# ut-amrl/nautilus

Measured on AMD Instinct MI355X. Metric: loop-closure candidate pairs/sec (1081-beam), higher is better.
Workload: dtype u16

## Files before the change

nautilus_amd/csm.py:

```python
import ctypes as C
import math

import numpy as np

from . import _lib
from ._lib import GridSpec, GridLayout, Search, Match, check, ptr

MATCH_DTYPE = np.dtype([("itheta", "<i4"), ("ix", "<i4"), ("iy", "<i4"), ("score", "<f4")])
assert MATCH_DTYPE.itemsize == C.sizeof(Match) == 16


def grid_spec(range_m=30.0, res=0.05, sigma=2.0, floor_p=1e-10, max_shift=40, cell_bits=16, skip_map=False, no_image=False):
    return GridSpec(float(range_m), float(res), float(sigma), float(floor_p), int(max_shift), int(cell_bits),
                    (_lib.NHIP_GRID_SKIP_MAP if skip_map else 0) | (_lib.NHIP_GRID_NO_IMAGE if no_image else 0), 0)


def search_spec(n_theta=61, nx=81, ny=81, theta_step=math.radians(1.0), exhaustive=False, dense=False, short_scans=False,
                exact_score=False, latency=False):
    flags = (_lib.NHIP_SEARCH_EXHAUSTIVE if exhaustive else 0) | (_lib.NHIP_SEARCH_DENSE if dense else 0) | \
            (_lib.NHIP_SEARCH_SHORT_SCANS if short_scans else 0) | (_lib.NHIP_SEARCH_EXACT_SCORE if exact_score else 0) | \
            (_lib.NHIP_SEARCH_LATENCY if latency else 0)
    return Search(int(n_theta), int(nx), int(ny), flags, float(theta_step))


def grid_layout(spec):
    out = GridLayout()
    check(_lib.load().nhip_grid_layout(C.byref(spec), C.byref(out)))
    return out


def angle_mod(a):
    return a - 2.0 * math.pi * np.rint(a / (2.0 * math.pi))


def rot0_table(rot_a, rot_b=None):
    rot_a = np.ascontiguousarray(rot_a, dtype=np.float64)
    rb = None if rot_b is None else np.ascontiguousarray(rot_b, dtype=np.float64)
    out = np.empty((rot_a.size, 2), dtype=np.float64)
    check(_lib.load().nhip_csm_rot0(ptr(rot_a), ptr(rb), rot_a.size, ptr(out)))
    return out


def delta_table(search):
    out = np.empty((search.n_theta, 2), dtype=np.float64)
    check(_lib.load().nhip_csm_delta_table(C.byref(search), ptr(out)))
    return out


def pack_scans(scans):
    offsets = np.zeros(len(scans) + 1, dtype=np.int32)
    for i, s in enumerate(scans):
        offsets[i + 1] = offsets[i] + len(s)
    xy = np.zeros((int(offsets[-1]), 2), dtype=np.float32)
    for i, s in enumerate(scans):
        if len(s):
            xy[offsets[i]:offsets[i + 1]] = np.asarray(s, dtype=np.float32).reshape(-1, 2)
    return xy, offsets


class ScanTable:

    def __init__(self, xy, offsets):
        self.xy = np.ascontiguousarray(xy, dtype=np.float32).reshape(-1, 2)
        self.offsets = np.ascontiguousarray(offsets, dtype=np.int32)
        self.n_scans = self.offsets.size - 1
        self._h = C.c_void_p()
        check(_lib.load().nhip_scans_upload(ptr(self.xy), ptr(self.offsets), self.n_scans, C.byref(self._h)))

    @classmethod
    def from_list(cls, scans):
        return cls(*pack_scans(scans))

    def close(self):
        if self._h:
            _lib.load().nhip_scans_free(self._h)
            self._h = C.c_void_p()

    __del__ = close


class LikelihoodGrids:

    def __init__(self, scans, target_ids, spec):
        self.spec = spec
        self.layout = grid_layout(spec)
        self.target_ids = np.ascontiguousarray(target_ids, dtype=np.int32)
        self._h = C.c_void_p()
        check(_lib.load().nhip_grids_build(scans._h, ptr(self.target_ids), self.target_ids.size,
                                           C.byref(spec), C.byref(self._h)))

    @classmethod
    def from_submaps(cls, scans, member_scan, member_affine, member_offsets, spec):
        self = cls.__new__(cls)
        self.spec = spec
        self.layout = grid_layout(spec)
        self.member_scan = np.ascontiguousarray(member_scan, dtype=np.int32)
        self.member_affine = np.ascontiguousarray(member_affine, dtype=np.float32).reshape(-1, 4)
        self.member_offsets = np.ascontiguousarray(member_offsets, dtype=np.int32)
        if self.member_offsets.size < 1 or len(self.member_affine) != self.member_scan.size:
            raise ValueError("from_submaps: one affine per member, n_targets + 1 offsets")
        self.target_ids = np.arange(self.member_offsets.size - 1, dtype=np.int32)
        self._h = C.c_void_p()
        check(_lib.load().nhip_grids_build_submaps(scans._h, ptr(self.member_scan), ptr(self.member_affine),
                                                   ptr(self.member_offsets), self.target_ids.size, C.byref(spec),
                                                   C.byref(self._h)))
        return self

    def was_rebuilt(self):
        return bool(_lib.load().nhip_grids_was_rebuilt(self._h))

    def download(self, slot):
        L = self.layout
        out = np.empty((L.rows, L.pitch), dtype=np.uint8)
        check(_lib.load().nhip_grids_download(self._h, int(slot), ptr(out)))
        return out.view(np.uint16) if L.cell_bytes == 2 else out

    def hi_plane(self, slot, copy=0):
        L = self.layout
        out = np.empty((L.rows, L.hi_pitch), dtype=np.uint8)
        check(_lib.load().nhip_grids_download_hi_plane_copy(self._h, int(slot), int(copy), ptr(out)))
        return out

    def tiled16(self, slot):
        L = self.layout
        out = np.empty((L.rows, L.pitch), dtype=np.uint8)
        check(_lib.load().nhip_grids_download_tiled16(self._h, int(slot), ptr(out)))
        return out.view(np.uint16)

    def skip_map(self, slot):
        L = self.layout
        out = np.empty(L.skip_bytes, dtype=np.uint8)
        check(_lib.load().nhip_grids_download_skip_map(self._h, int(slot), ptr(out)))
        mp = 8 * ((L.pitch // 4 + 63) // 64)
        return out[:L.rows * mp].reshape(L.rows, mp)

    def pooled(self, slot, level=1):
        L = self.layout
        if level == 1:
            out = np.empty((L.pool_rows, L.pool_pitch), dtype=np.uint8)
            check(_lib.load().nhip_grids_download_pool(self._h, int(slot), ptr(out)))
        else:
            out = np.empty((L.pool4_rows, L.pool4_pitch), dtype=np.uint8)
            check(_lib.load().nhip_grids_download_pool4(self._h, int(slot), ptr(out)))
        return out

    def hits(self, slot):
        L = self.layout
        raw = np.empty(L.hits_bytes, dtype=np.uint8)
        check(_lib.load().nhip_grids_download_hits(self._h, int(slot), ptr(raw)))
        rows = raw[:L.hits_pitch * (L.side + 64)].reshape(L.side + 64, L.hits_pitch)
        bits = np.unpackbits(rows, axis=1, bitorder="little")
        return bits[32:32 + L.side, 32:32 + L.side]

    def interior(self, slot):
        L = self.layout
        return self.download(slot)[L.pad:L.pad + L.side, L.pad:L.pad + L.side]

    def close(self):
        if self._h:
            _lib.load().nhip_grids_free(self._h)
            self._h = C.c_void_p()

    __del__ = close


def submap_member_affines(poses, anchor_of_member, member_scan):
    P = np.ascontiguousarray(poses, dtype=np.float64).reshape(-1, 3)
    a = np.ascontiguousarray(anchor_of_member, dtype=np.int32)
    m = np.ascontiguousarray(member_scan, dtype=np.int32)
    if a.size != m.size:
        raise ValueError("submap_member_affines: one anchor per member")
    out = np.empty((m.size, 4), dtype=np.float32)
    check(_lib.load().nhip_submap_member_affines(ptr(P), len(P), ptr(a), ptr(m), m.size, ptr(out)))
    return out


def match_pairs(scans, grids, pair_src, pair_slot, theta0, search, pair_origin=None, min_score=None):
    pair_src = np.ascontiguousarray(pair_src, dtype=np.int32)
    pair_slot = np.ascontiguousarray(pair_slot, dtype=np.int32)
    theta0 = np.ascontiguousarray(theta0, dtype=np.float64)
    n = pair_src.size
    if pair_slot.size != n or theta0.size != n:
        raise ValueError("pair arrays differ in length")
    org = None
    if pair_origin is not None:
        org = np.ascontiguousarray(pair_origin, dtype=np.int32).reshape(n, 2)
    out = np.zeros(n, dtype=MATCH_DTYPE)
    sums = np.zeros(n, dtype=np.int32)
    if min_score is None:
        check(_lib.load().nhip_csm_match(scans._h, grids._h, ptr(pair_src), ptr(pair_slot), ptr(theta0),
                                         ptr(org), n, C.byref(search), ptr(out), ptr(sums)))
    else:
        check(_lib.load().nhip_csm_match_gated(scans._h, grids._h, ptr(pair_src), ptr(pair_slot), ptr(theta0),
                                               ptr(org), n, C.byref(search), ptr(out), ptr(sums), float(min_score)))
    return out, sums


def rejected(matches):
    return np.asarray(matches)["itheta"] < 0


def gate_floor(spec, min_score, n_points):
    out = C.c_int32(0)
    check(_lib.load().nhip_csm_gate_floor(C.byref(spec), float(min_score), int(n_points), C.byref(out)))
    return out.value


def bnb_stats():
    a, b = C.c_uint64(0), C.c_uint64(0)
    check(_lib.load().nhip_bnb_stats(C.byref(a), C.byref(b)))
    return a.value, b.value


def bnb_stats_levels():
    v = (C.c_uint64 * 24)()
    check(_lib.load().nhip_bnb_stats_levels(v))
    return {"blocks_whole": v[0], "blocks_total": v[1], "candidates_refined": v[2], "sub_blocks": v[3],
            "clk_wave_phase3": v[4], "clk_origins": v[5], "clk_sub_bounds": v[6], "clk_exact": v[7],
            "clk_slowest_wave": v[8], "clk_seeds": v[9], "clk_bounds": v[10], "clk_wave_phase3_100MHz": v[11],
            "pairs_handed_over": v[12], "clk_wave_second_kernel": v[13], "pose_evals16": v[14],
            "pairs_settled_by_gate": v[15], "passes_l2_runs": v[16], "passes_per_cell_field": v[17],
            "passes_per_cell_capacity": v[18]}


def score_volume(scans, grids, src, slot, theta0, search, origin=(0, 0)):
    out = np.zeros((search.n_theta, search.nx, search.ny), dtype=np.int32)
    check(_lib.load().nhip_csm_scores(scans._h, grids._h, int(src), int(slot), float(theta0),
                                      int(origin[0]), int(origin[1]), C.byref(search), ptr(out)))
    return out


def match_to_transform(m, spec, search, theta0, origin=(0, 0)):
    tx = (origin[0] + int(m["ix"]) - (search.nx - 1) // 2) * spec.res
    ty = (origin[1] + int(m["iy"]) - (search.ny - 1) // 2) * spec.res
    th = theta0 + (int(m["itheta"]) - (search.n_theta - 1) // 2) * search.theta_step
    return np.float32(tx), np.float32(ty), np.float32(th)


class CorrelativeScanMatcher:

    def __init__(self, scanner_range, trans_range, low_res, high_res, sigma=2.0, cell_bits=16):
        self.params = _lib.CsmParams(float(scanner_range), float(trans_range), float(low_res), float(high_res),
                                     float(sigma), 1e-10, int(cell_bits), 0)

    def GetTransformation(self, pointcloud_a, pointcloud_b, rotation_a, rotation_b, rotation_restriction):
        a = np.ascontiguousarray(pointcloud_a, dtype=np.float32).reshape(-1, 2)
        b = np.ascontiguousarray(pointcloud_b, dtype=np.float32).reshape(-1, 2)
        score, tx, ty, th = C.c_double(0), C.c_float(0), C.c_float(0), C.c_float(0)
        check(_lib.load().nhip_csm_get_transformation(C.byref(self.params), ptr(a), len(a), ptr(b), len(b),
                                                      float(rotation_a), float(rotation_b), float(rotation_restriction),
                                                      C.byref(score), C.byref(tx), C.byref(ty), C.byref(th)))
        return score.value, ((np.float32(tx.value), np.float32(ty.value)), np.float32(th.value))


def last_launch():
    out = (C.c_int32 * 8)()
    check(_lib.load().nhip_csm_last_launch(out))
    form = {0: "fused", 1: "split, one round", 2: "split, rounds on one stream", 3: "split, rounds overlapped on the helper stream"}
    return {"form": form.get(out[0], "?"), "form_id": out[0], "pairs_per_round": out[1], "rounds_of_state": out[2],
            "rounds": out[3], "short_scans": bool(out[4]), "hand_over_kernel": bool(out[5]), "instrumented": bool(out[6] & 1),
            "l2_runs": bool(out[6] & 2), "n_pairs": out[7]}


def drop_in_cache_stats():
    v = [C.c_int64(0) for _ in range(4)]
    check(_lib.load().nhip_csm_cache_stats(*[C.byref(x) for x in v]))
    return dict(zip(("entries", "bytes", "hits", "misses"), (x.value for x in v)))


def drop_in_cache_clear():
    check(_lib.load().nhip_csm_cache_clear())


def drop_in_cache_configure(max_bytes):
    check(_lib.load().nhip_csm_cache_configure(int(max_bytes)))
```

nautilus_amd/csrc/nhip_bnb.hip:

```cpp
#include <atomic>
#include <mutex>
#include <type_traits>
#include <vector>

#ifndef NHIP_BNB_INSTR
#define NHIP_BNB_INSTR 0
#endif
#if NHIP_BNB_INSTR
#define csm_bnb_kernel csm_bnb_kernel_instr
#define csm_bnb_rot_kernel csm_bnb_rot_kernel_instr
#define launchers_product launchers_instr
#define BNB_STATS(P) ((P).stats)
#define BNB_TIMELINE(P) ((P).timeline)
#else
#define BNB_STATS(P) (static_cast<unsigned long long *>(nullptr))
#define BNB_TIMELINE(P) (static_cast<unsigned long long *>(nullptr))
#endif

#include "nhip_bnb_params.h"
#include "nhip_bnb_wave.h"
#include "nhip_bnb_origin.h"
#include "nhip_bnb_bounds.h"
#include "nhip_bnb_exact.h"

namespace nhip {

namespace {

using namespace bnb;

constexpr int BNB_THREADS = 64 * BNB_WAVES;

struct PairCtx {
  const uint8_t *grid;
  const float2 *pts;
  int32_t n_pts, cx, cy, pair;
};

template <int CB>
__device__ __forceinline__ void process_candidate(const BnbParams &P, const PairCtx &C, int32_t k, int32_t v, int lane,
                                                  unsigned long long *best, uint32_t (&n)[4]) {
  const int Y = v / NB, X = v - NB * Y;
  float cf, sf;
  rotation_k(P, C.pair, k, &cf, &sf);
  if (P.levels >= 2) {
    const __amdgpu_buffer_rsrc_t p4 = uniform_rsrc(C.grid + P.grid_bytes + P.skip_bytes + P.pool_bytes, P.pool4_bytes);
    uint32_t sb[4];
    sub_bounds(P, p4, C.pts, C.n_pts, cf, sf, C.cx, C.cy, Y, X, lane, CB == 1 ? 1u : 257u, sb);
    n[1]++;
    const uint32_t bsum = best_sum<false>(best);
    int alive = 0;
#pragma unroll
    for (int q = 0; q < 4; q++) alive += (sb[q] != 0u && sb[q] >= bsum) ? 1 : 0;
    if (alive == 0) return;
    if (alive <= 2) {
      const __amdgpu_buffer_rsrc_t rsrc = uniform_rsrc(C.grid, P.grid_bytes + P.skip_bytes);
#pragma unroll 1
      for (int q = 0; q < 4; q++) {
        const uint32_t b = q == 0 ? sb[0] : (q == 1 ? sb[1] : (q == 2 ? sb[2] : sb[3]));
        if (b == 0u || b < best_sum<false>(best)) continue;
        const unsigned long long key = eval_sub<CB>(P, rsrc, C.pts, C.n_pts, cf, sf, C.cx, C.cy, k, Y, X, q >> 1, q & 1, lane);
        wave_atomic_max(best, key, lane);
        n[2]++;
      }
      return;
    }
  }
  const unsigned long long key = eval_block<CB>(P, C.grid, C.pts, C.n_pts, cf, sf, C.cx, C.cy, k, Y, X, lane);
  wave_atomic_max(best, key, lane);
  n[0]++;
}

template <int CB, bool GLOBAL>
__device__ __forceinline__ void process_candidate_c(const BnbParams &P, __amdgpu_buffer_rsrc_t rsrc, uint32_t pitch8,
                                                    __amdgpu_buffer_rsrc_t rsrc16, const uint32_t *org, int32_t nch,
                                                    int32_t n_pts, int32_t k, int32_t Y, int32_t X,
                                                    uint32_t sb0, uint32_t sb1, uint32_t sb2, uint32_t sb3, int lane,
                                                    unsigned long long *best, uint32_t &bcopy, uint32_t (&n)[4]) {
  const uint32_t bsum = best_sum_cached<GLOBAL>(best, bcopy);
  const int alive = (sb0 != 0u && sb0 >= bsum) + (sb1 != 0u && sb1 >= bsum) + (sb2 != 0u && sb2 >= bsum) +
                    (sb3 != 0u && sb3 >= bsum);
  if (alive == 0) return;
  constexpr int WHOLE_MIN = 3;
  if (alive >= WHOLE_MIN) {
    int dy, dx;
    const uint32_t total = block_sums8(rsrc, pitch8, (uint32_t)P.hi_copy_bytes, org, nch, Y, X, lane, &dy, &dx);
    const int32_t ix = BNB_B * X + dx, iy = BNB_B * Y + dy;
    if (CB == 1) {
      const unsigned long long key = best_key(P, k, ix, iy, total, 32);
      wave_atomic_max(best, key, lane);
      if (GLOBAL) bcopy = max(bcopy, (uint32_t)(key >> 32));
    } else {
      n[3] += refine16<GLOBAL>(P, rsrc16, org, nch, n_pts, k, ix, iy, total, true, lane, best, bcopy);
    }
    n[0]++;
    return;
  }
#pragma unroll 1
  for (int q = 0; q < 4; q++) {
    const uint32_t b = q == 0 ? sb0 : (q == 1 ? sb1 : (q == 2 ? sb2 : sb3));
    if (b == 0u || b < best_sum_cached<GLOBAL>(best, bcopy)) continue;
    int dy, dx;
    const uint32_t total = sub_sums8(rsrc, pitch8, (uint32_t)P.hi_copy_bytes, org, nch, Y, X, q >> 1, q & 1, lane, &dy, &dx);
    const int32_t ix = BNB_B * X + BNB_B4 * (q & 1) + dx, iy = BNB_B * Y + BNB_B4 * (q >> 1) + dy;
    if (CB == 1) {
      const unsigned long long key = best_key(P, k, ix, iy, total, 8);
      wave_atomic_max(best, key, lane);
      if (GLOBAL) bcopy = max(bcopy, (uint32_t)(key >> 32));
    } else {
      n[3] += refine16<GLOBAL>(P, rsrc16, org, nch, n_pts, k, ix, iy, total, lane < 16, lane, best, bcopy);
    }
    n[2]++;
  }
}

struct PhaseClocks {
  long long org, strip, eval;
  uint32_t run_passes, cell_passes_field, cell_passes_full;
};

__device__ __forceinline__ void flush_stats(unsigned long long *stats, const uint32_t *n, int32_t pair, const PhaseClocks *clk) {
  if (n) {
    if (n[0]) atomicAdd(&stats[0], (unsigned long long)n[0]);
    if (n[1]) atomicAdd(&stats[2], (unsigned long long)n[1]);
    if (n[2]) atomicAdd(&stats[3], (unsigned long long)n[2]);
    if (n[3]) atomicAdd(&stats[14], (unsigned long long)n[3]);
    if (pair < BNB_STATS_PAIRS) atomicAdd(&stats[BNB_STATS_HEAD + pair], 4ull * n[0] + n[2]);
  }
  if (clk) {
    atomicAdd(&stats[5], (unsigned long long)clk->org);
    atomicAdd(&stats[6], (unsigned long long)clk->strip);
    atomicAdd(&stats[7], (unsigned long long)clk->eval);
    if (clk->run_passes) atomicAdd(&stats[16], (unsigned long long)clk->run_passes);
    if (clk->cell_passes_field) atomicAdd(&stats[17], (unsigned long long)clk->cell_passes_field);
    if (clk->cell_passes_full) atomicAdd(&stats[18], (unsigned long long)clk->cell_passes_full);
  }
}

template <int CB, bool GLOBAL, bool RUNS = false>
__device__ __forceinline__ void rotation_pass(const BnbParams &P, const PairCtx &C, int32_t k, uint32_t u0, uint32_t u1,
                                              unsigned long long m0, unsigned long long m1, int lane,
                                              unsigned long long *best, uint32_t *done, uint32_t *org,
                                              uint32_t (&n_work)[4], PhaseClocks &clk, uint32_t *runs = nullptr) {
  long long t_mark = 0;
  float cf, sf;
  rotation_k(P, C.pair, k, &cf, &sf);
  if (BNB_STATS(P)) t_mark = clock64();
  int32_t nrc = RUNS_NONE;
  const int32_t nch = cache_origins<RUNS>(P, C.pts, C.n_pts, cf, sf, C.cx, C.cy, lane, org, true, runs, RUNS && P.l2_runs != 0, &nrc);
  if (BNB_STATS(P)) clk.org += clock64() - t_mark;
  if (RUNS && BNB_STATS(P)) {
    clk.run_passes += nrc > 0 ? 1u : 0u;
    clk.cell_passes_field += nrc == RUNS_FIELD ? 1u : 0u;
    clk.cell_passes_full += nrc == RUNS_FULL ? 1u : 0u;
  }
  const __amdgpu_buffer_rsrc_t rsrc16 = CB == 1 ? uniform_rsrc(C.grid, P.grid_bytes + P.skip_bytes)
                                                : uniform_rsrc(C.grid + P.hi_offset + 2 * P.hi_copy_bytes, P.t16_bytes);
  const __amdgpu_buffer_rsrc_t rsrc = uniform_rsrc(C.grid + P.hi_offset, 2 * P.hi_copy_bytes);
  const uint32_t pitch8 = (uint32_t)P.hi_tpr;
  const __amdgpu_buffer_rsrc_t p4 = uniform_rsrc(C.grid + P.grid_bytes + P.skip_bytes + P.pool_bytes, P.pool4_bytes);
  while ((m0 | m1) != 0ull) {
    const int b0 = m0 ? (int)__builtin_ctzll(m0) : 64 + (int)__builtin_ctzll(m1);
    const int Y = b0 / NB, X0 = b0 - NB * Y;
    int len = 1;
    while (len < 3 && X0 + len < NB) {
      const int b = b0 + len;
      if (!(((b < 64 ? m0 >> b : m1 >> (b - 64)) & 1ull))) break;
      len++;
    }
    uint32_t sb[12];
    uint32_t bcopy = GLOBAL ? best_sum<true>(best) : 0u;
    if (P.levels >= 2) {
      if (BNB_STATS(P)) t_mark = clock64();
      if (RUNS && nrc > 0) strip_bounds_c<RunList<RUN_CHUNKS>>(P, p4, runs + lane, nrc, Y, X0, len, CB == 1 ? 1u : 257u, sb);
      else strip_bounds_c<CellList>(P, p4, org, nch, Y, X0, len, CB == 1 ? 1u : 257u, sb);
      if (BNB_STATS(P)) clk.strip += clock64() - t_mark;
      n_work[1] += (uint32_t)len;
    } else {
#pragma unroll
      for (int q = 0; q < 12; q++) sb[q] = 0xffffffffu;
    }
#pragma unroll 1
    for (int t = 0; t < len; t++) {
      const int b = b0 + t;
      if (b < 64) m0 &= ~(1ull << b);
      else m1 &= ~(1ull << (b - 64));
      const uint32_t ub = (uint32_t)__builtin_amdgcn_readlane((int)(b < 64 ? u0 : u1), b & 63);
      if (ub < best_sum_cached<GLOBAL>(best, bcopy)) continue;
      const uint32_t s0 = t == 0 ? sb[0] : (t == 1 ? sb[4] : sb[8]), s1 = t == 0 ? sb[1] : (t == 1 ? sb[5] : sb[9]);
      const uint32_t s2 = t == 0 ? sb[2] : (t == 1 ? sb[6] : sb[10]), s3 = t == 0 ? sb[3] : (t == 1 ? sb[7] : sb[11]);
      if (BNB_STATS(P)) t_mark = clock64();
      process_candidate_c<CB, GLOBAL>(P, rsrc, pitch8, rsrc16, org, nch, C.n_pts, k, Y, X0 + t, s0, s1, s2, s3, lane, best,
                                      bcopy, n_work);
      if (BNB_STATS(P)) clk.eval += clock64() - t_mark;
      if (done && wave_leader(lane)) done[b] = 0u;
    }
  }
}

__device__ __forceinline__ void read_entry(const RotEntry *ent, int32_t *pair, int32_t *k, unsigned long long *m0,
                                           unsigned long long *m1) {
  const unsigned long long w0 = ent->w[0], w1 = ent->w[1], w2 = ent->w[2], w3 = ent->w[3];
  *pair = (int32_t)(w0 >> 24);
  *k = (int32_t)(w0 & 0xffffffull);
  *m0 = w1 | (w2 << 41);
  *m1 = (w2 >> 23) | (w3 << 18);
}

__device__ __forceinline__ void pair_context(const BnbParams &P, int32_t pair, PairCtx *C) {
  const int32_t src = P.pair_src[pair], slot = P.pair_slot[pair];
  const int32_t beg = P.offsets[src];
  C->grid = P.grids + (size_t)slot * P.slot_bytes;
  C->pts = P.xy + beg;
  C->n_pts = P.offsets[src + 1] - beg;
  C->cx = P.pair_origin ? P.pair_origin[2 * pair] : 0;
  C->cy = P.pair_origin ? P.pair_origin[2 * pair + 1] : 0;
  C->pair = pair;
}

template <int CB, bool POOL_LDS, bool BY_ROT, bool SPLIT = false>
__global__ __launch_bounds__(SPLIT ? 64 * SPLIT_WAVES : BNB_THREADS, SPLIT ? SPLIT_WAVES / 2 : 4) void csm_bnb_kernel(BnbParams P) {
  constexpr int WAVES = SPLIT ? SPLIT_WAVES : BNB_WAVES, THREADS = 64 * WAVES;
  constexpr int QSPACE = lds_qspace(SPLIT);
  extern __shared__ __align__(16) uint8_t smem[];
  uint8_t *s_pool = smem;
  uint32_t *s_org = reinterpret_cast<uint32_t *>(smem);
  uint32_t *s_U = reinterpret_cast<uint32_t *>(smem + P.lds_first);
  unsigned long long *s_queue = reinterpret_cast<unsigned long long *>(s_U + (size_t)P.n_theta * 128);
  LdsTail *s_tail = reinterpret_cast<LdsTail *>(s_queue + QSPACE);
  unsigned long long *s_best = &s_tail->best, *s_slow = &s_tail->slow;
  uint32_t *s_cnt = s_tail->cnt, *s_qn = s_cnt + LDS_QN, *s_qhead = s_cnt + LDS_QHEAD, *s_top = &s_tail->top;
  uint32_t *s_list = reinterpret_cast<uint32_t *>(s_queue);
  static_assert(BNB_WAVES * LIST_ENTRIES * 4 <= QCAP * 4, "the run lists fit the first half of the queue");
  unsigned long long *s_kmax = s_queue + (SPLIT ? WAVES * LIST_ENTRIES / 2 : QCAP / 2);
  uint32_t *s_order = reinterpret_cast<uint32_t *>(s_kmax + MAX_ROT);
  static_assert(SPLIT_WAVES * LIST_ENTRIES * 4 + MAX_ROT * 12 <= QSPACE_SPLIT * 8 && MAX_ROT * 12 <= QCAP * 4, "lists, maxima and order fit");

  const uint32_t bid = blockIdx.x;
  const int32_t pair = (int32_t)((bid & 7u) * (uint32_t)P.pairs_per_xcd + (bid >> 3));
  if ((int32_t)(bid >> 3) >= P.pairs_per_xcd || pair >= P.n_pairs) return;
  const int lane = threadIdx.x & 63, wave = threadIdx.x >> 6;

  int32_t src = P.pair_src[pair], slot = P.pair_slot[pair];
  const bool ids_ok = pair_ids_ok(P.ids, src, slot, pair + P.pair_base, threadIdx.x == 0);
  if (!ids_ok) src = slot = 0;
  const int32_t beg = ids_ok ? P.offsets[src] : 0, n_pts = ids_ok ? P.offsets[src + 1] - beg : 0;
  const float2 *pts = P.xy + beg;
  const uint8_t *grid = P.grids + (size_t)slot * P.slot_bytes;
  const int32_t cx = P.pair_origin ? P.pair_origin[2 * pair] : 0;
  const int32_t cy = P.pair_origin ? P.pair_origin[2 * pair + 1] : 0;
  const bool centre_ok = (abs(cx) + P.hx <= P.max_shift) && (abs(cy) + P.hy <= P.max_shift);
  if (BY_ROT != (n_pts <= 64 * OCL && (uint32_t)P.rows < ORG_LIMIT && !P.general_all)) return;

  const int32_t gfloor = gate_floor(P.gate, n_pts);
  const unsigned long long fkey = gate_floor_key(gfloor);
  unsigned long long *const stats_g = NHIP_BNB_INSTR ? P.stats : nullptr;
  const long long t_start = BNB_STATS(P) ? clock64() : 0;
  if (BNB_TIMELINE(P) && threadIdx.x == 0 && pair < BNB_STATS_PAIRS) BNB_TIMELINE(P)[4 * pair] = wall_clock64();
  if (threadIdx.x == 0) {
    *s_slow = 0ull;
    *s_best = fkey;
    s_cnt[0] = s_cnt[3] = s_cnt[4] = s_cnt[5] = 0u;
    s_top[0] = 0u;
    *s_qn = 0u;
    *s_qhead = 0u;
  }
  if (!centre_ok || n_pts <= 0) {
    if (threadIdx.x == 0) P.keys[pair] = fkey;
    return;
  }
  if (POOL_LDS) {
    const uint4 *gp = reinterpret_cast<const uint4 *>(grid + P.grid_bytes + P.skip_bytes);
    uint4 *sp = reinterpret_cast<uint4 *>(s_pool);
    const int32_t n16 = (int32_t)(P.pool_bytes / 16);
    for (int32_t i = threadIdx.x; i < n16; i += 4 * THREADS) {
      uint4 v[4];
#pragma unroll
      for (int j = 0; j < 4; j++) v[j] = gp[min(i + j * THREADS, n16 - 1)];
#pragma unroll
      for (int j = 0; j < 4; j++)
        if (i + j * THREADS < n16) sp[i + j * THREADS] = v[j];
    }
  }
  const __amdgpu_buffer_rsrc_t prs = uniform_rsrc(grid + P.grid_bytes + P.skip_bytes, P.pool_bytes);
  __syncthreads();

  const uint32_t scale = CB == 1 ? 1u : 257u;
  unsigned long long wbest = 0ull;
  for (int32_t k = wave; k < P.n_theta; k += WAVES) {
    float cf, sf;
    rotation_k(P, pair, k, &cf, &sf);
    uint32_t umax = 0u;
    uint32_t tot[2];
    coarse_rotation<POOL_LDS>(P, s_pool, prs, pts, n_pts, cf, sf, cx, cy, lane, s_list + wave * LIST_ENTRIES, tot);
    if (lane < 128 - NB * NB) s_U[k * 128 + NB * NB + lane] = 0u;
#pragma unroll
    for (int i = 0; i < 2; i++) {
      int Y, X;
      if (!slot_block(lane + 64 * i, &Y, &X)) continue;
      const uint32_t u = (Y < P.nby && X < P.nbx) ? tot[i] * scale : 0u;
      const int b = NB * Y + X;
      s_U[k * 128 + b] = u;
      umax = u > umax ? u : umax;
      const unsigned long long cand = ((unsigned long long)u << 32) | (uint32_t)((k << 8) | b);
      wbest = cand > wbest ? cand : wbest;
    }
    if (BY_ROT) {
      umax = wave_max(umax);
      if (wave_leader(lane)) s_kmax[k] = ((unsigned long long)umax << 32) | (uint32_t)k;
    }
  }
  wbest = wave_max_u64(wbest);
  if (gfloor > 0) {
    if (wave_leader(lane)) atomicMax(s_top, (uint32_t)(wbest >> 32));
    __syncthreads();
    if (*s_top < (uint32_t)gfloor) {
      if (threadIdx.x == 0) {
        P.keys[pair] = fkey;
        if (stats_g) {
          atomicAdd(&stats_g[1], (unsigned long long)(P.n_theta * P.nbx * P.nby));
          atomicAdd(&stats_g[15], 1ull);
        }
      }
      return;
    }
    if ((uint32_t)(wbest >> 32) < (uint32_t)gfloor) wbest = 0ull;
  }
  uint32_t n_work[4] = {0u, 0u, 0u, 0u};
  PairCtx C;
  C.grid = grid;
  C.pts = pts;
  C.n_pts = n_pts;
  C.cx = cx;
  C.cy = cy;
  C.pair = pair;
  if (BY_ROT) {
    __syncthreads();
    uint32_t *org = s_org + wave * ORG_WAVE + lane;
    PhaseClocks clk = {0, 0, 0, 0u, 0u, 0u};
    long long t_busy = 0, t_wall = 0;
    const long long t_phase1 = BNB_STATS(P) ? clock64() : 0;
    if (BNB_TIMELINE(P) && threadIdx.x == 0 && pair < BNB_STATS_PAIRS) BNB_TIMELINE(P)[4 * pair + 1] = wall_clock64();
    const uint32_t xcd = bid & 7u;
    bool handed_over = false;
    enum { SEED, OWN };
    int state = SEED;
    bool heavy = false;
    for (;;) {
      bool have = false;
      int32_t k = 0;
      uint32_t u0 = 0u, u1 = 0u;
      unsigned long long m0 = 0ull, m1 = 0ull;
      uint32_t *done = nullptr;
      if (state == SEED) {
        if ((uint32_t)(wbest >> 32) != 0u) {
          const int32_t v = (int32_t)(wbest & 0xffu);
          const uint32_t ub = (uint32_t)(wbest >> 32);
          k = (int32_t)((uint32_t)wbest >> 8);
          u0 = v == lane ? ub : 0u;
          u1 = v == lane + 64 ? ub : 0u;
          m0 = v < 64 ? 1ull << v : 0ull;
          m1 = v < 64 ? 0ull : 1ull << (v - 64);
          done = s_U + k * 128;
          have = true;
        }
      } else if (state == OWN) {
        const int32_t rank = (int32_t)wave_fetch_add(s_qhead, 1u, lane);
        if (rank >= P.n_theta) break;
        k = (int32_t)s_order[rank];
        u0 = s_U[k * 128 + lane];
        u1 = s_U[k * 128 + 64 + lane];
        const uint32_t bsum = best_sum<false>(s_best);
        m0 = __ballot(u0 != 0u && u0 >= bsum);
        m1 = __ballot(u1 != 0u && u1 >= bsum && lane + 64 < NB * NB);
        if ((m0 | m1) == 0ull) continue;
        if (heavy && (uint32_t)rank >= P.keep_ranks) {
          const uint32_t lx = (xcd + (uint32_t)rank) & 7u;
          const uint32_t e = wave_fetch_add(P.rot_count + 8 * lx, 1u, lane);
          if (e < P.rot_cap) {
            if (lane < 4) {
              const unsigned long long M41 = (1ull << 41) - 1ull;
              const unsigned long long word = lane == 0   ? ((unsigned long long)(uint32_t)pair << 24) | (uint32_t)k
                                              : lane == 1 ? (m0 & M41)
                                              : lane == 2 ? ((m0 >> 41) | (m1 << 23)) & M41
                                                          : (m1 >> 18);
              P.rot_list[(size_t)lx * P.rot_cap + e].w[lane] = word;
            }
            handed_over = true;
            continue;
          }
        }
        have = true;
      }
      if (have) rotation_pass<CB, false>(P, C, k, u0, u1, m0, m1, lane, s_best, done, org, n_work, clk);
      if (state == SEED) {
        __syncthreads();
        if (BNB_TIMELINE(P) && threadIdx.x == 0 && pair < BNB_STATS_PAIRS) BNB_TIMELINE(P)[4 * pair + 2] = wall_clock64();
        if (BNB_STATS(P)) {
          t_busy = clock64();
          t_wall = wall_clock64();
        }
        for (int32_t kk = threadIdx.x; kk < P.n_theta; kk += THREADS) {
          const unsigned long long mine = s_kmax[kk];
          int32_t rank = 0;
          for (int32_t j = 0; j < P.n_theta; j++) rank += s_kmax[j] > mine ? 1 : 0;
          s_order[rank] = (uint32_t)kk;
        }
        if (P.rot_list || SPLIT) {
          const uint32_t bsum = best_sum<false>(s_best);
          uint32_t mine = 0u;
          for (int32_t kk = wave; kk < P.n_theta; kk += WAVES) {
            const uint32_t c0 = s_U[kk * 128 + lane], c1 = s_U[kk * 128 + 64 + lane];
            mine += (uint32_t)__builtin_popcountll(__ballot(c0 != 0u && c0 >= bsum)) +
                    (uint32_t)__builtin_popcountll(__ballot(c1 != 0u && c1 >= bsum && lane + 64 < NB * NB));
          }
          if (wave_leader(lane)) atomicAdd(s_qn, mine);
        }
        __syncthreads();
        if (SPLIT) {
          const uint32_t bsum = best_sum<false>(s_best);
          uint32_t *rows = P.ps_rows + (size_t)pair * (size_t)P.n_theta * 128u;
          uint32_t live = 0u;
          for (int32_t r = wave; r < P.n_theta; r += WAVES) {
            const uint32_t kk = s_order[r];
            const uint32_t kmax = (uint32_t)(s_kmax[kk] >> 32);
            if (kmax == 0u || kmax < bsum) break;
            live = (uint32_t)r + 1u;
            const uint32_t w1 = lane == 62 ? kmax : (lane == 63 ? kk : s_U[kk * 128 + 64 + lane]);
            rows[(size_t)r * 128u + lane] = s_U[kk * 128 + lane];
            rows[(size_t)r * 128u + 64 + lane] = w1;
          }
          if (live && wave_leader(lane)) atomicMax(s_qhead, live);
          __syncthreads();
          if (threadIdx.x == 0) {
            P.ps_count[pair] = *s_qn;
            P.ps_live[pair] = *s_qhead;
            P.ps_next[pair] = 0u;
          }
          break;
        }
        heavy = P.rot_list && *s_qn >= P.heavy_min;
        state = OWN;
      }
    }
    if (BNB_STATS(P) && lane == 0) {
      const long long now = clock64();
      atomicAdd(&BNB_STATS(P)[4], (unsigned long long)(now - t_busy));
      atomicAdd(&BNB_STATS(P)[11], (unsigned long long)(wall_clock64() - t_wall));
      flush_stats(BNB_STATS(P), nullptr, pair, &clk);
      atomicMax(s_slow, (unsigned long long)(now - t_busy));
      if (wave == 0) {
        atomicAdd(&BNB_STATS(P)[9], (unsigned long long)(t_busy - t_phase1));
        atomicAdd(&BNB_STATS(P)[10], (unsigned long long)(t_phase1 - t_start));
        if (handed_over) atomicAdd(&BNB_STATS(P)[12], 1ull);
      }
    }
  } else {
  if ((uint32_t)(wbest >> 32) != 0u) {
      const int32_t k = (int32_t)((uint32_t)wbest >> 8), v = (int32_t)(wbest & 0xffu);
      const int Y = v / NB, X = v - NB * Y;
      float cf, sf;
      rotation_k(P, pair, k, &cf, &sf);
      const unsigned long long key = eval_block<CB>(P, grid, pts, n_pts, cf, sf, cx, cy, k, Y, X, lane);
      if (wave_leader(lane)) {
        atomicMax(s_best, key);
        s_U[k * 128 + v] = 0u;
      }
      n_work[0]++;
    }
    __syncthreads();
    for (int32_t k = wave; k < P.n_theta; k += BNB_WAVES) {
  #pragma unroll
      for (int i = 0; i < 2; i++) {
        const uint32_t u = s_U[k * 128 + lane + 64 * i];
        const uint32_t bsum = (uint32_t)(*(volatile unsigned long long *)s_best >> 32);
        bool cand = u != 0u && u >= bsum;
        const unsigned long long m = __ballot(cand);
        if (m == 0ull) continue;
        const uint32_t base = wave_fetch_add(s_qn, (uint32_t)__builtin_popcountll(m), lane);
        const uint32_t pos = base + (uint32_t)__builtin_popcountll(m & ((1ull << lane) - 1ull));
        const unsigned long long entry = ((unsigned long long)u << 32) | (uint32_t)((k << 8) | (lane + 64 * i));
        if (cand && pos < (uint32_t)QCAP) s_queue[pos] = entry;
        unsigned long long over = __ballot(cand && pos >= (uint32_t)QCAP);
        while (over) {
          const int j = (int)__builtin_ctzll(over);
          over &= over - 1ull;
          const uint32_t lo = (uint32_t)__builtin_amdgcn_readlane((int)(uint32_t)entry, j);
          const uint32_t hi = (uint32_t)__builtin_amdgcn_readlane((int)(uint32_t)(entry >> 32), j);
          if (hi >= best_sum<false>(s_best))
            process_candidate<CB>(P, C, (int32_t)(lo >> 8), (int32_t)(lo & 0xffu), lane, s_best, n_work);
        }
      }
    }
    __syncthreads();
    {
      const uint32_t qn = min(*s_qn, (uint32_t)QCAP);
      for (;;) {
        const uint32_t i = wave_fetch_add(s_qhead, 1u, lane);
        if (i >= qn) break;
        const unsigned long long entry = s_queue[i];
        if ((uint32_t)(entry >> 32) >= best_sum<false>(s_best))
          process_candidate<CB>(P, C, (int32_t)((uint32_t)entry >> 8), (int32_t)(entry & 0xffu), lane, s_best, n_work);
      }
    }
}
  if (stats_g && lane == 0) {
    atomicAdd(&s_cnt[0], n_work[0]);
    atomicAdd(&s_cnt[3], n_work[1]);
    atomicAdd(&s_cnt[4], n_work[2]);
    atomicAdd(&s_cnt[5], n_work[3]);
  }
  __syncthreads();
  if (threadIdx.x == 0) {
    P.keys[pair] = *s_best;
    if (BNB_TIMELINE(P) && pair < BNB_STATS_PAIRS) {
      uint32_t hw;
      asm volatile("s_getreg_b32 %0, hwreg(HW_REG_HW_ID)" : "=s"(hw));
      uint32_t xcc;
      asm volatile("s_getreg_b32 %0, hwreg(HW_REG_XCC_ID)" : "=s"(xcc));
      BNB_TIMELINE(P)[4 * pair + 3] = (wall_clock64() & 0xfffffffffffull) | ((unsigned long long)((hw >> 8) & 0xffu) << 44) |
                                      ((unsigned long long)(xcc & 0xfu) << 52);
    }
    if (BNB_STATS(P) && BY_ROT) atomicAdd(&BNB_STATS(P)[8], *s_slow);
    if (stats_g) {
      const uint32_t n_all[4] = {s_cnt[0], s_cnt[3], s_cnt[4], s_cnt[5]};
      flush_stats(stats_g, n_all, pair, nullptr);
      atomicAdd(&stats_g[1], (unsigned long long)(P.n_theta * P.nbx * P.nby));
    }
  }
}

template <int CB>
__global__ __launch_bounds__(256, 4) void csm_bnb_rot_kernel(BnbParams P) {
  const int lane = threadIdx.x & 63;
  const uint32_t xcd = blockIdx.x & 7u;
  const uint32_t filled = P.rot_count[8 * xcd];
  const uint32_t count = filled < P.rot_cap ? filled : P.rot_cap;
  const RotEntry *list = P.rot_list + (size_t)xcd * P.rot_cap;
  __shared__ uint32_t s_org2[4 * ORG_WAVE];
  __shared__ uint32_t s_run2[4 * RUN_WAVE];
  uint32_t *org = s_org2 + (threadIdx.x >> 6) * ORG_WAVE + lane;
  uint32_t *runs = s_run2 + (threadIdx.x >> 6) * RUN_WAVE;
  PhaseClocks clk = {0, 0, 0, 0u, 0u, 0u};
  const long long t0 = BNB_STATS(P) ? clock64() : 0;
  for (;;) {
    const uint32_t i = wave_fetch_add(P.rot_count + 8 * xcd + 1, 1u, lane);
    if (i >= count) break;
    int32_t pair, k;
    unsigned long long m0, m1;
    read_entry(list + i, &pair, &k, &m0, &m1);
    PairCtx C;
    pair_context(P, pair, &C);
    uint32_t n[4] = {0u, 0u, 0u, 0u};
    rotation_pass<CB, true, true>(P, C, k, 0xffffffffu, 0xffffffffu, m0, m1, lane, &P.keys[pair], nullptr, org, n, clk, runs);
    if (BNB_STATS(P) && lane == 0) flush_stats(BNB_STATS(P), n, pair, nullptr);
  }
  if (BNB_STATS(P) && lane == 0) {
    atomicAdd(&BNB_STATS(P)[13], (unsigned long long)(clock64() - t0));
    flush_stats(BNB_STATS(P), nullptr, 0, &clk);
  }
}

constexpr int SORT_THREADS = 1024;
constexpr int SORT_BUCKETS = 16 * 21;
__device__ __forceinline__ int cand_bucket(uint32_t c) {
  if (c == 0u) return SORT_BUCKETS - 1;
  const int e = 31 - __builtin_clz(c);
  const int f = e >= 4 ? (int)((c >> (e - 4)) & 15u) : (int)((c << (4 - e)) & 15u);
  const int b = 16 * e + f;
  return b >= SORT_BUCKETS - 1 ? 0 : SORT_BUCKETS - 2 - b;
}
__device__ __forceinline__ uint32_t cand_shares(const BnbParams &P, uint32_t c) {
  const uint32_t w = 1u + c / P.split_min;
  return w < P.split_max ? w : P.split_max;
}

__global__ __launch_bounds__(SORT_THREADS) void csm_bnb_order_kernel(BnbParams P) {
  __shared__ uint32_t s_extra[SORT_BUCKETS];
  __shared__ uint32_t s_wave[SORT_THREADS / 64];
  __shared__ uint32_t s_base, s_idle;
  __shared__ int s_grant;
  const int32_t xcd = blockIdx.x;
  const int32_t lo = xcd * P.pairs_per_xcd, hi = min(lo + P.pairs_per_xcd, P.n_pairs);
  int32_t *work = P.ps_work + (size_t)xcd * P.ps_work_stride;
  for (int i = threadIdx.x; i < SORT_BUCKETS; i += SORT_THREADS) s_extra[i] = 0u;
  for (int i = threadIdx.x; i < P.ps_work_stride; i += SORT_THREADS) work[i] = -1;
  if (threadIdx.x == 0) s_base = s_idle = 0u;
  __syncthreads();
  for (int32_t p = lo + (int32_t)threadIdx.x; p < hi; p += SORT_THREADS) {
    const uint32_t c = P.ps_count[p];
    atomicAdd(&s_extra[cand_bucket(c)], cand_shares(P, c) - 1u);
  }
  __syncthreads();
  if (threadIdx.x == 0) {
    uint32_t room = (uint32_t)P.ps_work_stride - (uint32_t)(hi > lo ? hi - lo : 0);
    int grant = 0;
    while (grant < SORT_BUCKETS && s_extra[grant] <= room) room -= s_extra[grant++];
    s_grant = grant;
  }
  __syncthreads();
  const int lane = threadIdx.x & 63, wv = threadIdx.x >> 6;
  for (int pass = P.front_min ? 0 : 1; pass < 2; pass++)
  for (int32_t p0 = lo; p0 < hi; p0 += SORT_THREADS) {
    const int32_t p = p0 + (int32_t)threadIdx.x;
    const uint32_t c = p < hi ? P.ps_count[p] : 0u;
    const bool mine = P.front_min == 0u || ((c >= P.front_min) == (pass == 0));
    const uint32_t w = (c != 0u && mine) ? (cand_bucket(c) < s_grant ? cand_shares(P, c) : 1u) : 0u;
    if (p < hi && mine) P.ps_nw[p] = c != 0u ? w : 1u;
    uint32_t v = w;
#pragma unroll
    for (int off = 1; off < 64; off <<= 1) {
      const uint32_t u = (uint32_t)__shfl_up((int)v, off, 64);
      if (lane >= off) v += u;
    }
    if (lane == 63) s_wave[wv] = v;
    __syncthreads();
    uint32_t before = s_base;
    for (int q = 0; q < wv; q++) before += s_wave[q];
    const uint32_t at = before + v - w;
    for (uint32_t j = 0; j < w; j++) work[at + j] = p;
    __syncthreads();
    if (threadIdx.x == SORT_THREADS - 1) s_base = before + v;
    __syncthreads();
  }
  const uint32_t tail0 = s_base;
  for (int32_t p = lo + (int32_t)threadIdx.x; p < hi; p += SORT_THREADS)
    if (P.ps_count[p] == 0u) work[tail0 + atomicAdd(&s_idle, 1u)] = p;
}

constexpr int ORDER_THREADS = 256;
__global__ __launch_bounds__(ORDER_THREADS) void csm_bnb_order_spread_kernel(BnbParams P) {
  const int32_t p = (int32_t)(blockIdx.x * ORDER_THREADS + threadIdx.x);
  if (p >= P.n_pairs) return;
  const int32_t extra_slots = P.ps_work_stride - P.pairs_per_xcd;
  const int32_t home = p / P.pairs_per_xcd;
  P.ps_work[(size_t)home * P.ps_work_stride + extra_slots + (p - home * P.pairs_per_xcd)] = p;
  const uint32_t want = cand_shares(P, P.ps_count[p]) - 1u;
  uint32_t got = 0u;
  if (want) {
    const uint32_t t0 = atomicAdd(P.ps_ticket, want);
    for (uint32_t j = 0; j < want; j++) {
      const uint32_t e = t0 + j;
      if ((int32_t)(e >> 3) >= extra_slots) break;
      P.ps_work[(size_t)((e + (uint32_t)home + 1u) & 7u) * P.ps_work_stride + (e >> 3)] = p;
      got++;
    }
  }
  P.ps_nw[p] = 1u + got;
}

constexpr int CAND_WAVES = 4;
constexpr int CAND_THREADS = 64 * CAND_WAVES;
template <int CB>
__global__ __launch_bounds__(CAND_THREADS, CB == 2 ? 5 : 4) void csm_bnb_cand_kernel(BnbParams P) {
  __shared__ uint32_t s_org2[CAND_WAVES * ORG_WAVE];
  __shared__ uint32_t s_run2[CAND_WAVES * RUN_WAVE];
  __shared__ unsigned long long s_best2;
  __shared__ uint32_t s_next2;
  const int lane = threadIdx.x & 63;
  const uint32_t xcd = blockIdx.x & 7u, slot = blockIdx.x >> 3;
  if ((int32_t)slot >= P.ps_work_stride) return;
  const int32_t pair = P.ps_work[(size_t)xcd * P.ps_work_stride + slot];
  if (pair < 0) return;
  const uint32_t live = P.ps_live[pair];
  if (live == 0u) return;
  const bool shared = P.ps_nw[pair] > 1u;
  if (BNB_TIMELINE(P) && threadIdx.x == 0 && pair < BNB_STATS_PAIRS)
    atomicMin(&BNB_TIMELINE(P)[4 * (size_t)BNB_STATS_PAIRS + 2 + pair], wall_clock64());
  if (threadIdx.x == 0) {
    s_best2 = P.keys[pair];
    s_next2 = 0u;
  }
  __syncthreads();
  unsigned long long *best = shared ? &P.keys[pair] : &s_best2;
  uint32_t *next = shared ? &P.ps_next[pair] : &s_next2;
  const uint32_t *rows = P.ps_rows + (size_t)pair * (size_t)P.n_theta * 128u;
  uint32_t *org = s_org2 + (threadIdx.x >> 6) * ORG_WAVE + lane;
  uint32_t *runs = s_run2 + (threadIdx.x >> 6) * RUN_WAVE;
  PairCtx C;
  pair_context(P, pair, &C);
  uint32_t n_work[4] = {0u, 0u, 0u, 0u};
  PhaseClocks clk = {0, 0, 0, 0u, 0u, 0u};
  const long long t0 = BNB_STATS(P) ? clock64() : 0;
  for (;;) {
    const uint32_t rank = wave_fetch_add(next, 1u, lane);
    if (rank >= live) break;
    const uint32_t u0 = rows[(size_t)rank * 128u + lane], u1 = rows[(size_t)rank * 128u + 64 + lane];
    const uint32_t kmax = (uint32_t)__builtin_amdgcn_readlane((int)u1, 62);
    const int32_t k = __builtin_amdgcn_readlane((int)u1, 63);
    const uint32_t bsum = best_sum<true>(best);
    if (kmax < bsum) break;
    const unsigned long long m0 = __ballot(u0 != 0u && u0 >= bsum);
    const unsigned long long m1 = __ballot(u1 != 0u && u1 >= bsum && lane + 64 < NB * NB);
    if ((m0 | m1) == 0ull) continue;
    rotation_pass<CB, true, true>(P, C, k, u0, u1, m0, m1, lane, best, nullptr, org, n_work, clk, runs);
  }
  if (BNB_STATS(P) && lane == 0) {
    atomicAdd(&BNB_STATS(P)[13], (unsigned long long)(clock64() - t0));
    flush_stats(BNB_STATS(P), n_work, pair, &clk);
  }
  if (BNB_TIMELINE(P) && lane == 0 && pair < BNB_STATS_PAIRS)
    atomicMax(&BNB_TIMELINE(P)[5 * (size_t)BNB_STATS_PAIRS + 2 + pair], wall_clock64());
  if (!shared) {
    __syncthreads();
    if (threadIdx.x == 0) P.keys[pair] = s_best2;
  }
}

}

namespace bnb {

namespace {
template <int CB, bool PL, bool BR, bool SP = false>
int launch_main(const BnbParams &P, const BnbPlan &plan, hipStream_t s) {
  constexpr int THREADS = SP ? 64 * SPLIT_WAVES : BNB_THREADS;
  const size_t lds = lds_bytes((size_t)plan.lds_first, P.n_theta, SP);
  const int64_t blocks = (int64_t)P.pairs_per_xcd * 8;
  constexpr int MAX_DEV = 64;
  static std::atomic<size_t> lds_set[MAX_DEV];
  int dev = 0;
  if (hipGetDevice(&dev) != hipSuccess || dev < 0 || dev >= MAX_DEV) dev = -1;
  if (dev < 0 || lds > lds_set[dev].load(std::memory_order_relaxed)) {
    NHIP_TRY_HIP(hipFuncSetAttribute(reinterpret_cast<const void *>(csm_bnb_kernel<CB, PL, BR, SP>),
                                     hipFuncAttributeMaxDynamicSharedMemorySize, (int)lds));
    if (dev >= 0) lds_set[dev].store(lds, std::memory_order_relaxed);
  }
  hipLaunchKernelGGL((csm_bnb_kernel<CB, PL, BR, SP>), dim3((uint32_t)blocks), dim3(THREADS), lds, s, P);
  return NHIP_OK;
}

template <int CB, bool PL>
int launch_split_a(const BnbParams &P, const BnbPlan &plan, hipStream_t s) {
  int rc = launch_main<CB, PL, true, true>(P, plan, s);
  if (rc) return rc;
  if (!P.short_scans && (rc = launch_main<CB, PL, false>(P, plan, s))) return rc;
  if (P.ps_ticket)
    hipLaunchKernelGGL(csm_bnb_order_spread_kernel, dim3((uint32_t)((P.n_pairs + ORDER_THREADS - 1) / ORDER_THREADS)), dim3(ORDER_THREADS), 0, s, P);
  else
    hipLaunchKernelGGL(csm_bnb_order_kernel, dim3(8), dim3(SORT_THREADS), 0, s, P);
  return NHIP_OK;
}

template <int CB, bool PL>
int launch_both(const BnbParams &P, const BnbPlan &plan, hipStream_t s) {
  if (!P.general_all) {
    int rc = launch_main<CB, PL, true>(P, plan, s);
    if (rc) return rc;
    if (P.short_scans) return NHIP_OK;
  }
  return launch_main<CB, PL, false>(P, plan, s);
}

template <class F>
int with_instantiation(const BnbPlan &plan, F f) {
  using CB1 = std::integral_constant<int, 1>;
  using CB2 = std::integral_constant<int, 2>;
  if (plan.cb == 1) return plan.pool_lds ? f(CB1{}, std::true_type{}) : f(CB1{}, std::false_type{});
  return plan.pool_lds ? f(CB2{}, std::true_type{}) : f(CB2{}, std::false_type{});
}

int launch_fused(const BnbParams &P, const BnbPlan &plan, hipStream_t s) {
  return with_instantiation(plan, [&](auto cb, auto pl) {
    const int rc = launch_both<decltype(cb)::value, decltype(pl)::value>(P, plan, s);
    if (rc) return rc;
    if (plan.second) {
      const uint32_t rot_blocks = 256 * 4;
      hipLaunchKernelGGL(csm_bnb_rot_kernel<decltype(cb)::value>, dim3(rot_blocks), dim3(256), 0, s, P);
    }
    return NHIP_OK;
  });
}

int launch_split_bounds(const BnbParams &P, const BnbPlan &plan, hipStream_t s) {
  return with_instantiation(plan, [&](auto cb, auto pl) { return launch_split_a<decltype(cb)::value, decltype(pl)::value>(P, plan, s); });
}

int launch_split_cands(const BnbParams &P, const BnbPlan &plan, hipStream_t s) {
  return with_instantiation(plan, [&](auto cb, auto) {
    hipLaunchKernelGGL(csm_bnb_cand_kernel<decltype(cb)::value>, dim3((uint32_t)(8 * P.ps_work_stride)), dim3(CAND_THREADS), 0, s, P);
    return NHIP_OK;
  });
}
}

BnbLaunchers launchers_product() { return {launch_fused, launch_split_bounds, launch_split_cands}; }

}


}
```

nautilus_amd/csrc/nhip_bnb_bounds.h:

```cpp
#pragma once
#include <type_traits>

#include "nhip_bnb_origin.h"

namespace nhip {
namespace {

constexpr uint32_t LANE_WEIGHT = 64u;

template <bool POOL_LDS>
__device__ __forceinline__ void coarse_rotation(const BnbParams &P, const uint8_t *pool, __amdgpu_buffer_rsrc_t prs,
                                                const float2 *pts, int32_t n_pts, float cf, float sf, int32_t cx,
                                                int32_t cy, int lane, uint32_t *list, uint32_t (&tot)[2]) {
  const int32_t DP = P.pool_pitch;
  const uint32_t zero_a = (uint32_t)(((P.rows + BNB_B - 1) / BNB_B) * DP);
  tot[0] = tot[1] = 0u;
  uint32_t E[NB][3], O[NB][3];
#pragma unroll
  for (int y = 0; y < NB; y++)
#pragma unroll
    for (int d = 0; d < 3; d++) E[y][d] = O[y][d] = 0u;
  uint32_t head = 0u, tail = 0u;
  uint32_t reduced = 0u;
  uint32_t weight = 0u;

  auto gather = [&](uint32_t a, uint32_t cnt) {
    const uint32_t se = __umul24(a & 3u, 0x10001u) + 0x0c020c00u, so = se + 0x00010001u;
    const uint32_t *q = reinterpret_cast<const uint32_t *>(pool + (a & ~3u));
#pragma unroll
    for (int y = 0; y < NB; y++) {
      uint32_t w0, w1, w2, w3;
      if (POOL_LDS) {
        const uint32_t *row = q + (y * DP) / 4;
        w0 = row[0]; w1 = row[1]; w2 = row[2]; w3 = row[3];
      } else {
        const u32x4 r4 = __builtin_amdgcn_raw_buffer_load_b128(prs, (int)((a & ~3u) + (uint32_t)(y * DP)), 0, 0);
        w0 = r4.x; w1 = r4.y; w2 = r4.z; w3 = r4.w;
      }
      E[y][0] += __umul24(__builtin_amdgcn_perm(w1, w0, se), cnt); O[y][0] += __umul24(__builtin_amdgcn_perm(w1, w0, so), cnt);
      E[y][1] += __umul24(__builtin_amdgcn_perm(w2, w1, se), cnt); O[y][1] += __umul24(__builtin_amdgcn_perm(w2, w1, so), cnt);
      E[y][2] += __umul24(__builtin_amdgcn_perm(w3, w2, se), cnt); O[y][2] = mad24(__builtin_amdgcn_perm(w3, w2, so), cnt, O[y][2]);
    }
  };
  auto reduce = [&]() {
    uint32_t R[64];
#pragma unroll
    for (int y = 0; y < 10; y++)
#pragma unroll
      for (int d = 0; d < 3; d++) {
        R[6 * y + d] = E[y][d];
        R[6 * y + 3 + d] = O[y][d];
      }
    R[5] = (O[0][2] & 0xffffu) | (O[10][1] << 16);
    R[11] = (O[1][2] & 0xffffu) | (O[10][1] & 0xffff0000u);
    R[17] = (O[2][2] & 0xffffu) | (O[10][2] << 16);
    R[60] = E[10][0];
    R[61] = E[10][1];
    R[62] = E[10][2];
    R[63] = O[10][0];
    rs_step<64, 1>(R, lane & 1);
    rs_step<32, 2>(R, lane & 2);
    uint32_t V[32];
#pragma unroll
    for (int i = 0; i < 16; i++) {
      V[2 * i] = R[i] & 0xffffu;
      V[2 * i + 1] = R[i] >> 16;
    }
    rs_step<32, 4>(V, lane & 4);
    rs_step<16, 8>(V, lane & 8);
    rs_step<8, 16>(V, lane & 16);
    rs_step<4, 32>(V, lane & 32);
    tot[0] += V[0];
    tot[1] += V[1];
#pragma unroll
    for (int y = 0; y < NB; y++)
#pragma unroll
      for (int d = 0; d < 3; d++) E[y][d] = O[y][d] = 0u;
  };

  auto feed = [&](uint32_t a, int32_t c, bool more) {
    if (more) {
      const bool live = c + lane < n_pts;
      const uint32_t prev = (uint32_t)__builtin_amdgcn_update_dpp((int)a, (int)a, 0x138 , 0xF, 0xF, false);
      const bool is_head = (lane & 63) == 0 || a != prev;
      const unsigned long long H = __builtin_amdgcn_uicmp(a, prev, 33 ) | 1ull;
      uint32_t cnt = (uint32_t)(c + lane) & 127u;
      cnt += 1u;
      const int32_t n_live = n_pts - c;
      const unsigned long long He = H & (n_live >= 64 ? ~0ull : (1ull << n_live) - 1ull);
      if (is_head && live) {
        const uint32_t before = __builtin_amdgcn_mbcnt_hi((uint32_t)(He >> 32), __builtin_amdgcn_mbcnt_lo((uint32_t)He, 0u));
        list[(tail + before) & (LIST_ENTRIES - 1)] = a | ((cnt - 1u) << RUN_SHIFT);
      }
      tail += (uint32_t)__builtin_popcountll(He);
      __builtin_amdgcn_fence(__ATOMIC_RELEASE, "wavefront");
      __builtin_amdgcn_wave_barrier();
    }
    if (!more) {
      if (lane == 0) list[tail & (LIST_ENTRIES - 1)] = ((uint32_t)n_pts & 127u) << RUN_SHIFT;
      __builtin_amdgcn_fence(__ATOMIC_RELEASE, "wavefront");
      __builtin_amdgcn_wave_barrier();
    }
    for (;;) {
      const uint32_t avail = tail - head;
      if (avail < 65u && more) break;
      const bool last = avail == 0u;
      const bool mine = (uint32_t)lane < avail;
      const uint32_t entry = mine ? list[(head + (uint32_t)lane) & (LIST_ENTRIES - 1)] : zero_a;
      const uint32_t ea = entry & ((1u << RUN_SHIFT) - 1u);
      const uint32_t next = mine ? list[(head + (uint32_t)lane + 1u) & (LIST_ENTRIES - 1)] : 0u;
      const uint32_t cnt = mine ? ((next >> RUN_SHIFT) - (entry >> RUN_SHIFT)) & 127u : 0u;
      uint32_t left = avail;
      asm("" : "+s"(left));
      if (head != reduced && (left == 0u || __builtin_amdgcn_uicmp(weight + cnt, LANE_WEIGHT, 34 ) != 0ull)) {
        reduce();
        reduced = head;
        weight = 0u;
      }
      if (last) break;
      gather(ea, cnt);
      weight += cnt;
      head += avail < 64u ? avail : 64u;
      __builtin_amdgcn_wave_barrier();
    }
  };

  auto offsets = [&](float2 pt, int32_t c) {
    uint32_t a = zero_a;
    if (c + lane < n_pts) {
      int32_t prow, pcol;
      window_origin<true>(pt, cf, sf, P, cx, cy, &prow, &pcol);
      a = __umul24((uint32_t)prow >> 3, (uint32_t)DP) + ((uint32_t)pcol >> 3);
    }
    return a;
  };
  constexpr int PD = 2;
  if (n_pts > 0) {
    const int32_t last = n_pts - 1;
    float2 q0 = pts[min(lane, last)];
    __builtin_amdgcn_sched_barrier(0);
    float2 q1 = pts[min(64 + lane, last)];
    for (int32_t c = 0; c < n_pts; c += 64 * PD) {
      {
        float2 pt = q0;
        asm volatile("" : "+v"(pt.x), "+v"(pt.y));
        q0 = pts[min(c + 64 * PD + lane, last)];
        feed(offsets(pt, c), c, true);
      }
      {
        float2 pt = q1;
        asm volatile("" : "+v"(pt.x), "+v"(pt.y));
        q1 = pts[min(c + 64 * PD + 64 + lane, last)];
        if (c + 64 < n_pts) feed(offsets(pt, c + 64), c + 64, true);
      }
    }
  }
  feed(zero_a, 0, false);
}

__device__ __forceinline__ bool slot_block(int v, int *Y, int *X) {
  const int lane = v & 63, i = v >> 6;
  const int r = 32 * i + 16 * ((lane >> 5) & 1) + 8 * ((lane >> 4) & 1) + 4 * ((lane >> 3) & 1) + 2 * ((lane >> 1) & 1) + (lane & 1);
  const int f = (lane >> 2) & 1;
  if (r >= 60) {
    *Y = 10;
    *X = r == 63 ? 1 + 2 * f : 4 * (r - 60) + 2 * f;
    return true;
  }
  const int y = r / 6, d = r % 6;
  if (d == 5 && f == 1) {
    *Y = 10;
    *X = 5 + 2 * y;
    return y < 3;
  }
  *Y = y;
  *X = d < 3 ? 4 * d + 2 * f : 4 * (d - 3) + 1 + 2 * f;
  return true;
}

__device__ __forceinline__ void sub_bounds(const BnbParams &P, __amdgpu_buffer_rsrc_t p4, const float2 *pts, int32_t n_pts,
                                           float cf, float sf, int32_t cx, int32_t cy, int32_t Y, int32_t X, int lane,
                                           uint32_t scale, uint32_t (&out)[4]) {
  const int32_t DP = P.pool4_pitch;
  uint32_t A[4] = {0u, 0u, 0u, 0u};
  constexpr int U = 4;
  for (int32_t c = 0; c < n_pts; c += 64 * U) {
    uint32_t a[U];
    u32x2 w[U];
#pragma unroll
    for (int u = 0; u < U; u++) {
      const int32_t idx = c + 64 * u + lane;
      a[u] = 0u;
      if (idx < n_pts) {
        int32_t prow, pcol;
        window_origin(pts[idx], cf, sf, P, cx, cy, &prow, &pcol);
        a[u] = (uint32_t)(((prow >> 2) + 2 * Y) * DP + 2 * ((pcol >> 2) + 2 * X));
      }
      w[u] = __builtin_amdgcn_raw_buffer_load_b64(p4, (int)(a[u] & ~3u), 0, 0);
    }
#pragma unroll
    for (int u = 0; u < U; u++) {
      const uint32_t n = idx_guard(c + 64 * u + lane < n_pts, __builtin_amdgcn_alignbit(w[u].y, w[u].x, (a[u] & 2u) * 8u));
      A[0] += n & 0xffu;
      A[2] += (n >> 8) & 0xffu;
      A[1] += (n >> 16) & 0xffu;
      A[3] += n >> 24;
    }
  }
#pragma unroll
  for (int m = 1; m < 64; m <<= 1) {
#pragma unroll
    for (int q = 0; q < 4; q++) A[q] += shfl_xor_u32(A[q], m);
  }
#pragma unroll
  for (int q = 0; q < 4; q++) out[q] = A[q] * scale;
}

struct CellList {
  static constexpr int ROUNDS = 2, H = OC / ROUNDS;
  static __device__ __forceinline__ uint32_t entry(const uint32_t *list, int c) { return origin_of(list, c); }
  static __device__ __forceinline__ uint32_t offset(uint32_t o, uint32_t DP) { return (org_row(o) >> 2) * DP + 2u * (org_col(o) >> 2); }
  static __device__ __forceinline__ uint32_t count(uint32_t o) { return org_cnt(o); }
};
template <int CHUNKS>
struct RunList {
  static constexpr int ROUNDS = 1, H = CHUNKS;
  static __device__ __forceinline__ uint32_t entry(const uint32_t *list, int c) { return list[64 * c]; }
  static __device__ __forceinline__ uint32_t offset(uint32_t e, uint32_t DP) { return run_row2(e) * DP + 2u * run_col2(e); }
  static __device__ __forceinline__ uint32_t count(uint32_t e) { return run_cnt(e); }
};

template <class LIST>
__device__ __forceinline__ void strip_sums(const BnbParams &P, __amdgpu_buffer_rsrc_t p4, const uint32_t *list, int32_t nch,
                                           int32_t Y, int32_t X0, int len, uint32_t (&E)[3], uint32_t (&O)[3]) {
  const uint32_t DP = (uint32_t)P.pool4_pitch;
  const uint32_t off = (uint32_t)(2 * Y) * DP + (uint32_t)(4 * X0);
  constexpr int ROUNDS = LIST::ROUNDS, H = LIST::H;
#pragma unroll
  for (int h = 0; h < ROUNDS; h++) {
    if (H * h >= nch) continue;
    u32x4 w[H];
    uint32_t sh[H], cn[H];
    uint32_t aa[H];
#pragma unroll
    for (int j = 0; j < H; j++) {
      const uint32_t o = LIST::entry(list, H * h + j);
      const uint32_t a = LIST::offset(o, DP) + off;
      sh[j] = (a & 2u) * 8u;
      aa[j] = a & ~3u;
      cn[j] = LIST::count(o);
    }
    if (len == 1) {
#pragma unroll
      for (int j = 0; j < H; j++) {
        const u32x2 v = __builtin_amdgcn_raw_buffer_load_b64(p4, (int)aa[j], 0, 0);
        w[j].x = v.x; w[j].y = v.y; w[j].z = 0u; w[j].w = 0u;
      }
    } else if (len == 2) {
#pragma unroll
      for (int j = 0; j < H; j++) {
        const u32x3 v = __builtin_amdgcn_raw_buffer_load_b96(p4, (int)aa[j], 0, 0);
        w[j].x = v.x; w[j].y = v.y; w[j].z = v.z; w[j].w = 0u;
      }
    } else {
#pragma unroll
      for (int j = 0; j < H; j++) w[j] = __builtin_amdgcn_raw_buffer_load_b128(p4, (int)aa[j], 0, 0);
    }
#pragma unroll
    for (int j = 0; j < H; j++) {
      const uint32_t n0 = __builtin_amdgcn_alignbit(w[j].y, w[j].x, sh[j]);
      const uint32_t n1 = __builtin_amdgcn_alignbit(w[j].z, w[j].y, sh[j]);
      const uint32_t n2 = __builtin_amdgcn_alignbit(w[j].w, w[j].z, sh[j]);
      E[0] += __umul24(n0 & M8, cn[j]); O[0] += __umul24((n0 >> 8) & M8, cn[j]);
      E[1] += __umul24(n1 & M8, cn[j]); O[1] += __umul24((n1 >> 8) & M8, cn[j]);
      E[2] += __umul24(n2 & M8, cn[j]); O[2] += __umul24((n2 >> 8) & M8, cn[j]);
    }
  }
}

template <class LIST>
__device__ __forceinline__ void strip_bounds_c(const BnbParams &P, __amdgpu_buffer_rsrc_t p4, const uint32_t *list,
                                               int32_t nch, int32_t Y, int32_t X0, int len, uint32_t scale,
                                               uint32_t (&out)[12]) {
  uint32_t E[3] = {0u, 0u, 0u}, O[3] = {0u, 0u, 0u};
  if (std::is_same<LIST, CellList>::value) {
    strip_sums<CellList>(P, p4, list, nch, Y, X0, len, E, O);
  } else {
    static_assert(RUN_CHUNKS == 8, "the rounds below cover the run list");
    if (nch <= 4) strip_sums<RunList<4>>(P, p4, list, nch, Y, X0, len, E, O);
    else if (nch == 5) strip_sums<RunList<5>>(P, p4, list, nch, Y, X0, len, E, O);
    else if (nch == 6) strip_sums<RunList<6>>(P, p4, list, nch, Y, X0, len, E, O);
    else strip_sums<RunList<8>>(P, p4, list, nch, Y, X0, len, E, O);
  }
#pragma unroll
  for (int t = 0; t < 3; t++) {
    E[t] = sum8(E[t]);
    O[t] = sum8(O[t]);
  }
#pragma unroll
  for (int t = 0; t < 3; t++) {
    out[4 * t + 0] = E[t] & 0xffffu;
    out[4 * t + 1] = E[t] >> 16;
    out[4 * t + 2] = O[t] & 0xffffu;
    out[4 * t + 3] = O[t] >> 16;
  }
#pragma unroll
  for (int q = 0; q < 12; q++) out[q] = wave_total_of8(out[q]) * scale;
}

}
}
```

nautilus_amd/csrc/nhip_bnb_exact.h:

```cpp
#pragma once
#include "nhip_bnb_origin.h"

namespace nhip {
namespace {

constexpr int SEG_CHUNKS = 32;
constexpr int EVAL_CHUNKS = 2;

template <bool GLOBAL>
__device__ __forceinline__ uint32_t best_sum(unsigned long long *best) {
  unsigned long long b;
  if (GLOBAL) b = __hip_atomic_load(best, __ATOMIC_RELAXED, __HIP_MEMORY_SCOPE_AGENT);
  else b = *(volatile unsigned long long *)best;
  return (uint32_t)__builtin_amdgcn_readfirstlane((int)(uint32_t)(b >> 32));
}
template <bool GLOBAL>
__device__ __forceinline__ uint32_t best_sum_cached(unsigned long long *best, uint32_t copy) {
  return GLOBAL ? copy : best_sum<false>(best);
}

__device__ __forceinline__ unsigned long long best_key(const BnbParams &P, int32_t k, int32_t ix, int32_t iy, uint32_t total,
                                                       int top) {
  unsigned long long key = 0ull;
  if (ix < P.nx && iy < P.ny) {
    const uint32_t lin = (uint32_t)((k * P.nx + ix) * P.ny + iy);
    key = ((unsigned long long)total << 32) | (0xffffffffu - lin);
  }
#pragma unroll
  for (int m = 32; m >= 1; m >>= 1) {
    if (m > top) continue;
    const unsigned long long o = shfl_xor_u64b(key, m);
    key = o > key ? o : key;
  }
  return key;
}

template <int CB>
__device__ __forceinline__ unsigned long long eval_block(const BnbParams &P, const uint8_t *grid, const float2 *pts,
                                                         int32_t n_pts, float cf, float sf, int32_t cx, int32_t cy,
                                                         int32_t k, int32_t Y, int32_t X, int lane) {
  uint32_t total = 0u;
  int dy, dx;
  const __amdgpu_buffer_rsrc_t rsrc = uniform_rsrc(grid, P.grid_bytes + P.skip_bytes);
  if (CB == 1) {
    const float2 none = make_float2(0.f, 0.f);
    for (int32_t c0 = 0; c0 < n_pts; c0 += 64 * SEG_CHUNKS) {
      uint32_t E[8][2], O[8][2];
#pragma unroll
      for (int y = 0; y < 8; y++) E[y][0] = E[y][1] = O[y][0] = O[y][1] = 0u;
      const int32_t c1 = min(n_pts, c0 + 64 * SEG_CHUNKS);
      float qx[EVAL_CHUNKS], qy[EVAL_CHUNKS];
#pragma unroll
      for (int u = 0; u < EVAL_CHUNKS; u++) {
        const float2 q = c0 + 64 * u + lane < c1 ? pts[c0 + 64 * u + lane] : none;
        qx[u] = q.x;
        qy[u] = q.y;
      }
      for (int32_t c = c0; c < c1; c += 64 * EVAL_CHUNKS) {
        float nx[EVAL_CHUNKS], ny[EVAL_CHUNKS];
#pragma unroll
        for (int u = 0; u < EVAL_CHUNKS; u++) {
          const int32_t idx = c + 64 * (EVAL_CHUNKS + u) + lane;
          const float2 q = idx < c1 ? pts[idx] : none;
          nx[u] = q.x;
          ny[u] = q.y;
        }
        uint32_t g[EVAL_CHUNKS], sh[EVAL_CHUNKS], w[EVAL_CHUNKS][8][3];
#pragma unroll
        for (int u = 0; u < EVAL_CHUNKS; u++) {
          const int32_t idx = c + 64 * u + lane;
          patch_origin(P, idx < c1, make_float2(qx[u], qy[u]), cf, sf, cx, cy, Y, X, &g[u], &sh[u]);
#pragma unroll
          for (int y = 0; y < 8; y++) {
            const u32x3 r = __builtin_amdgcn_raw_buffer_load_b96(rsrc, (int)(g[u] + (uint32_t)(y * P.pitch)), 0, 0);
            w[u][y][0] = r.x; w[u][y][1] = r.y; w[u][y][2] = r.z;
          }
        }
#pragma unroll
        for (int u = 0; u < EVAL_CHUNKS; u++) {
#pragma unroll
          for (int y = 0; y < 8; y++) {
            const uint32_t n0 = __builtin_amdgcn_alignbit(w[u][y][1], w[u][y][0], sh[u]);
            const uint32_t n1 = __builtin_amdgcn_alignbit(w[u][y][2], w[u][y][1], sh[u]);
            E[y][0] += n0 & M8; O[y][0] += n0 >> 8;
            E[y][1] += n1 & M8; O[y][1] += n1 >> 8;
          }
          qx[u] = nx[u];
          qy[u] = ny[u];
        }
      }
      uint32_t R[32];
#pragma unroll
      for (int y = 0; y < 8; y++) {
        R[4 * y + 0] = E[y][0];
        R[4 * y + 1] = O[y][0] - ((E[y][0] >> 16) << 8);
        R[4 * y + 2] = E[y][1];
        R[4 * y + 3] = O[y][1] - ((E[y][1] >> 16) << 8);
      }
      rs_step<32, 1>(R, lane & 1);
      rs_step<16, 2>(R, lane & 2);
      rs_step<8, 4>(R, lane & 4);
      uint32_t V[8];
#pragma unroll
      for (int i = 0; i < 4; i++) {
        V[2 * i] = R[i] & 0xffffu;
        V[2 * i + 1] = R[i] >> 16;
      }
      rs_step<8, 8>(V, lane & 8);
      rs_step<4, 16>(V, lane & 16);
      rs_step<2, 32>(V, lane & 32);
      total += V[0];
    }
    const int r = 8 * (2 * ((lane >> 5) & 1) + ((lane >> 4) & 1)) + 4 * ((lane >> 2) & 1) + 2 * ((lane >> 1) & 1) + (lane & 1);
    const int f = (lane >> 3) & 1, d = r & 3;
    dy = r >> 2;
    dx = 4 * (d >> 1) + (d & 1) + 2 * f;
  } else {
    uint32_t A[64];
#pragma unroll
    for (int i = 0; i < 64; i++) A[i] = 0u;
    float2 qn = lane < n_pts ? pts[lane] : make_float2(0.f, 0.f);
    for (int32_t c = 0; c < n_pts; c += 64) {
      const float2 q = qn;
      if (c + 64 + lane < n_pts) qn = pts[c + 64 + lane];
      uint32_t g = 0u, sh = 0u;
      if (c + lane < n_pts) {
        int32_t prow, pcol;
        window_origin(q, cf, sf, P, cx, cy, &prow, &pcol);
        const int32_t col = pcol + BNB_B * X;
        g = (uint32_t)((prow + BNB_B * Y) * P.pitch + ((2 * col) & ~3));
        sh = (uint32_t)(col & 1) * 16u;
      }
#pragma unroll
      for (int y = 0; y < 8; y++) {
        const u32x4 r4 = __builtin_amdgcn_raw_buffer_load_b128(rsrc, (int)(g + (uint32_t)(y * P.pitch)), 0, 0);
        const uint32_t w[5] = {r4.x, r4.y, r4.z, r4.w,
                               __builtin_amdgcn_raw_buffer_load_b32(rsrc, (int)(g + (uint32_t)(y * P.pitch) + 16u), 0, 0)};
#pragma unroll
        for (int j = 0; j < 4; j++) {
          const uint32_t nj = __builtin_amdgcn_alignbit(w[j + 1], w[j], sh);
          A[8 * y + 2 * j] += nj & 0xffffu;
          A[8 * y + 2 * j + 1] += nj >> 16;
        }
      }
    }
    rs_step<64, 1>(A, lane & 1);
    rs_step<32, 2>(A, lane & 2);
    rs_step<16, 4>(A, lane & 4);
    rs_step<8, 8>(A, lane & 8);
    rs_step<4, 16>(A, lane & 16);
    rs_step<2, 32>(A, lane & 32);
    total = A[0];
    dy = lane >> 3;
    dx = lane & 7;
  }
  const int32_t ix = BNB_B * X + dx, iy = BNB_B * Y + dy;
  unsigned long long key = 0ull;
  if (ix < P.nx && iy < P.ny) {
    const uint32_t lin = (uint32_t)((k * P.nx + ix) * P.ny + iy);
    key = ((unsigned long long)total << 32) | (0xffffffffu - lin);
  }
#pragma unroll
  for (int m = 32; m >= 1; m >>= 1) {
    const unsigned long long o = shfl_xor_u64b(key, m);
    key = o > key ? o : key;
  }
  return key;
}

template <int CB>
__device__ __forceinline__ unsigned long long eval_sub(const BnbParams &P, __amdgpu_buffer_rsrc_t rsrc, const float2 *pts,
                                                       int32_t n_pts, float cf, float sf, int32_t cx, int32_t cy,
                                                       int32_t k, int32_t Y, int32_t X, int32_t sy, int32_t sx, int lane) {
  uint32_t total = 0u;
  int dy, dx;
  const float2 none = make_float2(0.f, 0.f);
  constexpr int U = 4;
  if (CB == 1) {
    static_assert(SEG_CHUNKS % U == 0, "segments are whole iterations");
    for (int32_t c0 = 0; c0 < n_pts; c0 += 64 * SEG_CHUNKS) {
      uint32_t E[4], O[4];
#pragma unroll
      for (int y = 0; y < 4; y++) E[y] = O[y] = 0u;
      const int32_t c1 = min(n_pts, c0 + 64 * SEG_CHUNKS);
      for (int32_t c = c0; c < c1; c += 64 * U) {
        uint32_t sh[U];
        u32x2 w[U][4];
#pragma unroll
        for (int u = 0; u < U; u++) {
          const int32_t idx = c + 64 * u + lane;
          uint32_t g;
          patch_origin(P, idx < c1, idx < c1 ? pts[idx] : none, cf, sf, cx, cy, Y, X, &g, &sh[u]);
          if (idx < c1) g += (uint32_t)(BNB_B4 * sy * P.pitch + BNB_B4 * sx);
#pragma unroll
          for (int y = 0; y < 4; y++) w[u][y] = __builtin_amdgcn_raw_buffer_load_b64(rsrc, (int)(g + (uint32_t)(y * P.pitch)), 0, 0);
        }
#pragma unroll
        for (int u = 0; u < U; u++)
#pragma unroll
          for (int y = 0; y < 4; y++) {
            const uint32_t n = __builtin_amdgcn_alignbit(w[u][y].y, w[u][y].x, sh[u]);
            E[y] += n & M8;
            O[y] += n >> 8;
          }
      }
      uint32_t R[8];
#pragma unroll
      for (int y = 0; y < 4; y++) {
        R[2 * y] = E[y];
        R[2 * y + 1] = O[y] - ((E[y] >> 16) << 8);
      }
      rs_step<8, 1>(R, lane & 1);
      rs_step<4, 2>(R, lane & 2);
      rs_step<2, 4>(R, lane & 4);
      uint32_t V[2] = {R[0] & 0xffffu, R[0] >> 16};
      rs_step<2, 8>(V, lane & 8);
      V[0] = add_xor<16>(V[0]);
      V[0] = add_xor<32>(V[0]);
      total += V[0];
    }
    dy = ((lane >> 1) & 1) + 2 * ((lane >> 2) & 1);
    dx = (lane & 1) + 2 * ((lane >> 3) & 1);
  } else {
    uint32_t A[16];
#pragma unroll
    for (int i = 0; i < 16; i++) A[i] = 0u;
    for (int32_t c = 0; c < n_pts; c += 64 * U) {
      uint32_t sh[U];
      u32x3 w[U][4];
#pragma unroll
      for (int u = 0; u < U; u++) {
        const int32_t idx = c + 64 * u + lane;
        uint32_t g = 0u;
        sh[u] = 0u;
        if (idx < n_pts) {
          int32_t prow, pcol;
          window_origin(pts[idx], cf, sf, P, cx, cy, &prow, &pcol);
          const int32_t col = pcol + BNB_B * X + BNB_B4 * sx;
          g = (uint32_t)((prow + BNB_B * Y + BNB_B4 * sy) * P.pitch + ((2 * col) & ~3));
          sh[u] = (uint32_t)(col & 1) * 16u;
        }
#pragma unroll
        for (int y = 0; y < 4; y++) w[u][y] = __builtin_amdgcn_raw_buffer_load_b96(rsrc, (int)(g + (uint32_t)(y * P.pitch)), 0, 0);
      }
#pragma unroll
      for (int u = 0; u < U; u++)
#pragma unroll
        for (int y = 0; y < 4; y++) {
          const uint32_t n0 = __builtin_amdgcn_alignbit(w[u][y].y, w[u][y].x, sh[u]);
          const uint32_t n1 = __builtin_amdgcn_alignbit(w[u][y].z, w[u][y].y, sh[u]);
          A[4 * y + 0] += n0 & 0xffffu;
          A[4 * y + 1] += n0 >> 16;
          A[4 * y + 2] += n1 & 0xffffu;
          A[4 * y + 3] += n1 >> 16;
        }
    }
    rs_step<16, 1>(A, lane & 1);
    rs_step<8, 2>(A, lane & 2);
    rs_step<4, 4>(A, lane & 4);
    rs_step<2, 8>(A, lane & 8);
    A[0] = add_xor<16>(A[0]);
    A[0] = add_xor<32>(A[0]);
    total = A[0];
    dy = (lane >> 2) & 3;
    dx = lane & 3;
  }
  const int32_t ix = BNB_B * X + BNB_B4 * sx + dx, iy = BNB_B * Y + BNB_B4 * sy + dy;
  unsigned long long key = 0ull;
  if (ix < P.nx && iy < P.ny) {
    const uint32_t lin = (uint32_t)((k * P.nx + ix) * P.ny + iy);
    key = ((unsigned long long)total << 32) | (0xffffffffu - lin);
  }
#pragma unroll
  for (int m = 8; m >= 1; m >>= 1) {
    const unsigned long long o = shfl_xor_u64b(key, m);
    key = o > key ? o : key;
  }
  return key;
}

__device__ __forceinline__ uint32_t sub_sums8(__amdgpu_buffer_rsrc_t rsrc, uint32_t pitch, uint32_t copy_bytes, const uint32_t *org,
                                              int32_t nch, int32_t Y, int32_t X, int32_t sy, int32_t sx, int lane, int *dy, int *dx) {
  const uint32_t roff = (uint32_t)(BNB_B * Y + BNB_B4 * sy), coff = (uint32_t)(BNB_B * X + BNB_B4 * sx);
  const uint32_t wrap = pitch * HI_TILE_BYTES - HI_TILE_BYTES;
  constexpr int U = 2;
  static_assert(OC % U == 0, "whole rounds");
  uint32_t E[4] = {0u, 0u, 0u, 0u}, O[4] = {0u, 0u, 0u, 0u};
#pragma unroll
  for (int r = 0; r < OC / U; r++) {
    if (U * r >= nch) continue;
    u32x2 w[U][4];
    uint32_t sh[U], cn[U];
#pragma unroll
    for (int j = 0; j < U; j++) {
      const uint32_t o = origin_of(org, U * r + j);
      cn[j] = org_cnt(o);
      const uint32_t row0 = org_row(o) + roff, col0 = org_col(o) + coff, col4 = col0 & ~3u;
      const uint32_t cp = (col4 >> 3) & 1u, q = row0 & 7u;
      const uint32_t v0 = hi_tiled(row0, col4, cp, pitch, copy_bytes);
      sh[j] = (col0 & 3u) * 8u;
#pragma unroll
      for (int y = 0; y < 4; y++)
        w[j][y] = __builtin_amdgcn_raw_buffer_load_b64(rsrc, (int)(v0 + (q + (uint32_t)y >= 8u ? wrap : 0u) + 16u * (uint32_t)y), 0, 0);
    }
#pragma unroll
    for (int j = 0; j < U; j++)
#pragma unroll
      for (int y = 0; y < 4; y++) {
        const uint32_t n = __builtin_amdgcn_alignbit(w[j][y].y, w[j][y].x, sh[j]);
        E[y] += __umul24(n & M8, cn[j]);
        O[y] += __umul24(n >> 8, cn[j]);
      }
  }
  uint32_t R[8];
#pragma unroll
  for (int y = 0; y < 4; y++) {
    R[2 * y] = E[y];
    R[2 * y + 1] = O[y] - ((E[y] >> 16) << 8);
  }
  rs_step<8, 1>(R, lane & 1);
  rs_step<4, 2>(R, lane & 2);
  rs_step<2, 4>(R, lane & 4);
  uint32_t V[2] = {R[0] & 0xffffu, R[0] >> 16};
  rs_step<2, 8>(V, lane & 8);
  V[0] = add_xor<16>(V[0]);
  V[0] = add_xor<32>(V[0]);
  *dy = ((lane >> 1) & 1) + 2 * ((lane >> 2) & 1);
  *dx = (lane & 1) + 2 * ((lane >> 3) & 1);
  return V[0];
}

__device__ __forceinline__ uint32_t block_sums8(__amdgpu_buffer_rsrc_t rsrc, uint32_t pitch, uint32_t copy_bytes, const uint32_t *org,
                                                int32_t nch, int32_t Y, int32_t X, int lane, int *dy, int *dx) {
  const uint32_t roff = (uint32_t)(BNB_B * Y), coff = (uint32_t)(BNB_B * X);
  const uint32_t wrap = pitch * HI_TILE_BYTES - HI_TILE_BYTES;
  constexpr int U = 1;
  uint32_t E[8][2], O[8][2];
#pragma unroll
  for (int y = 0; y < 8; y++) E[y][0] = E[y][1] = O[y][0] = O[y][1] = 0u;
#pragma unroll
  for (int r = 0; r < OC / U; r++) {
    if (U * r >= nch) continue;
    constexpr int ROWS = 4;
    uint32_t gg[U], sh[U], cn[U], qq[U];
#pragma unroll
    for (int j = 0; j < U; j++) {
      const uint32_t o = origin_of(org, U * r + j);
      cn[j] = org_cnt(o);
      const uint32_t row0 = org_row(o) + roff, col0 = org_col(o) + coff, col4 = col0 & ~3u;
      qq[j] = row0 & 7u;
      gg[j] = hi_tiled(row0, col4, (col4 >> 3) & 1u, pitch, copy_bytes);
      sh[j] = (col0 & 3u) * 8u;
    }
#pragma unroll
    for (int y0 = 0; y0 < 8; y0 += ROWS) {
      u32x3 w[U][ROWS];
#pragma unroll
      for (int j = 0; j < U; j++)
#pragma unroll
        for (int y = 0; y < ROWS; y++)
          w[j][y] = __builtin_amdgcn_raw_buffer_load_b96(rsrc, (int)(gg[j] + (qq[j] + (uint32_t)(y0 + y) >= 8u ? wrap : 0u) + 16u * (uint32_t)(y0 + y)), 0, 0);
#pragma unroll
      for (int j = 0; j < U; j++)
#pragma unroll
        for (int y = 0; y < ROWS; y++) {
          const uint32_t n0 = __builtin_amdgcn_alignbit(w[j][y].y, w[j][y].x, sh[j]);
          const uint32_t n1 = __builtin_amdgcn_alignbit(w[j][y].z, w[j][y].y, sh[j]);
          E[y0 + y][0] += __umul24(n0 & M8, cn[j]); O[y0 + y][0] += __umul24(n0 >> 8, cn[j]);
          E[y0 + y][1] += __umul24(n1 & M8, cn[j]); O[y0 + y][1] += __umul24(n1 >> 8, cn[j]);
        }
    }
  }
  uint32_t R[32];
#pragma unroll
  for (int y = 0; y < 8; y++) {
    R[4 * y + 0] = E[y][0];
    R[4 * y + 1] = O[y][0] - ((E[y][0] >> 16) << 8);
    R[4 * y + 2] = E[y][1];
    R[4 * y + 3] = O[y][1] - ((E[y][1] >> 16) << 8);
  }
  rs_step<32, 1>(R, lane & 1);
  rs_step<16, 2>(R, lane & 2);
  rs_step<8, 4>(R, lane & 4);
  uint32_t V[8];
#pragma unroll
  for (int i = 0; i < 4; i++) {
    V[2 * i] = R[i] & 0xffffu;
    V[2 * i + 1] = R[i] >> 16;
  }
  rs_step<8, 8>(V, lane & 8);
  rs_step<4, 16>(V, lane & 16);
  rs_step<2, 32>(V, lane & 32);
  const int r = 8 * (2 * ((lane >> 5) & 1) + ((lane >> 4) & 1)) + 4 * ((lane >> 2) & 1) + 2 * ((lane >> 1) & 1) + (lane & 1);
  const int f = (lane >> 3) & 1, d = r & 3;
  *dy = r >> 2;
  *dx = 4 * (d >> 1) + (d & 1) + 2 * f;
  return V[0];
}

__device__ __forceinline__ uint32_t pose_sum16(const BnbParams &P, __amdgpu_buffer_rsrc_t rsrc16, const uint32_t *org,
                                               int32_t nch, int32_t ix, int32_t iy) {
  uint32_t acc = 0u;
#pragma unroll
  for (int c = 0; c < OCL; c++) {
    if (c >= nch) continue;
    const uint32_t o = origin_of(org, c);
    acc += org_cnt(o) * (uint32_t)__builtin_amdgcn_raw_buffer_load_b16(
                            rsrc16, (int)t16_tiled(org_row(o) + (uint32_t)iy, org_col(o) + (uint32_t)ix, (uint32_t)P.t16_tpr), 0, 0);
  }
  return wave_sum(acc);
}

template <bool GLOBAL>
__device__ __forceinline__ uint32_t refine16(const BnbParams &P, __amdgpu_buffer_rsrc_t rsrc16, const uint32_t *org,
                                             int32_t nch, int32_t n_pts, int32_t k, int32_t ix, int32_t iy, uint32_t hsum,
                                             bool mine, int lane, unsigned long long *best, uint32_t &bcopy) {
  const bool valid = mine && ix < P.nx && iy < P.ny;
  uint32_t ub = valid ? 256u * hsum + 255u * (uint32_t)n_pts : 0u;
  uint32_t n_eval = 0u;
  for (;;) {
    const uint32_t top = (uint32_t)__builtin_amdgcn_readfirstlane((int)wave_max(ub));
    if (top == 0u || top < best_sum_cached<GLOBAL>(best, bcopy)) break;
    const int j = (int)__builtin_ctzll(__ballot(ub == top));
    const int32_t jx = __builtin_amdgcn_readlane(ix, j), jy = __builtin_amdgcn_readlane(iy, j);
    const uint32_t sum = pose_sum16(P, rsrc16, org, nch, jx, jy);
    const uint32_t lin = (uint32_t)((k * P.nx + jx) * P.ny + jy);
    const unsigned long long key = ((unsigned long long)sum << 32) | (0xffffffffu - lin);
    wave_atomic_max(best, key, lane);
    if (GLOBAL) bcopy = max(bcopy, sum);
    if (lane == j) ub = 0u;
    n_eval++;
  }
  return n_eval;
}

}
}
```

nautilus_amd/csrc/nhip_bnb_host.hip:

```cpp
#include <atomic>
#include <memory>
#include <mutex>
#include <vector>

#include "nhip_bnb_params.h"

namespace nhip {

using namespace bnb;

namespace {

size_t bnb_lds_first(const GridLayout &L, bool pool_lds) {
  const size_t pool = pool_lds ? (size_t)L.pool_bytes : 0;
  return pool > (size_t)ORG_LDS ? pool : (size_t)ORG_LDS;
}
size_t bnb_lds_bytes(const GridLayout &L, const nhip_search_t *search, bool pool_lds) {
  return lds_bytes(bnb_lds_first(L, pool_lds), search->n_theta, false);
}
constexpr size_t LDS_MAX = 160 * 1024;

struct TimerScope {
  int id;
  hipStream_t s;
  TimerScope(int i, hipStream_t st) : id(i), s(st) { timer_begin(id, s); }
  ~TimerScope() { timer_end(id, s); }
};
}

bool bnb_fits(const GridLayout &L, const nhip_search_t *search) {
  const int nbx = (search->nx + BNB_B - 1) / BNB_B, nby = (search->ny + BNB_B - 1) / BNB_B;
  return nbx <= NB && nby <= NB && bnb_lds_bytes(L, search, false) <= LDS_MAX && L.pool_bytes % 16 == 0 &&
         L.pool_bytes < (1ll << RUN_SHIFT) && L.S + 2 * L.pad < 65536 && search->n_theta <= MAX_ROT;
}

static std::mutex g_instr_mu;
static unsigned long long *g_bnb_timeline = nullptr;
static unsigned long long *g_bnb_stats = nullptr;

constexpr int64_t BNB_WS_HEADER = 256;
constexpr int64_t SPLIT_PAIRS = 131072, SPLIT_MIN_PAIRS = 192, SPLIT_RING = 16;
constexpr int64_t SPREAD_BELOW_PAIRS = 4096;
constexpr int64_t SPLIT_SLOT_FIXED = 8 * 64 * 4 + 1024;
constexpr uint32_t FRONT_MIN = 64;

static int64_t split_state_bytes(int64_t pairs, int64_t batches, int32_t n_theta) {
  return batches * SPLIT_SLOT_FIXED + pairs * (16 + 6 + (int64_t)n_theta * 512);
}
static uint32_t bnb_split_max(int64_t nb) { return nb < SPREAD_BELOW_PAIRS ? 16u : (nb >= 8192 ? 4u : 8u); }

int64_t bnb_workspace_bytes_lists(int32_t n_pairs) {
  const int64_t n = n_pairs > 0 ? n_pairs : 0;
  return BNB_WS_HEADER + 8 * (((n + 7) / 8) * 16 + 64) * (int64_t)sizeof(RotEntry);
}
int64_t bnb_workspace_bytes(int32_t n_pairs) {
  const int64_t n = n_pairs > 0 ? n_pairs : 0;
  nhip_search_t any = {};
  const int64_t m = n <= SPLIT_PAIRS ? n : 2 * SPLIT_PAIRS;
  const int64_t split = bnb_plan(GridLayout(), &any, (int32_t)n, 0).sized_split
                            ? BNB_WS_HEADER + split_state_bytes(m, m / 512 + 4, 64) : 0;
  return std::max(bnb_workspace_bytes_lists(n_pairs), split);
}

BnbPlan bnb_plan(const GridLayout &L, const nhip_search_t *search, int32_t n_pairs, int64_t workspace_bytes) {
  const auto is = [](const char *v, char c) { return v && v[0] == c; };
  const auto num = [](const char *name, int unset) { const char *v = tunable(name); return v ? atoi(v) : unset; };
  const char *force = tunable("NHIP_BNB_KERNELS");
  const char *sp = tunable("NHIP_BNB_SPLIT");
  const char *sbat = tunable("NHIP_BNB_SPLIT_BATCH");
  const char *smax = tunable("NHIP_BNB_SPLIT_MAX");
  BnbPlan p = {};
  p.n_pairs = n_pairs;
  p.cb = L.cb;
  p.levels = is(tunable("NHIP_BNB_LEVELS"), '1') ? 1 : 2;
  p.l2_runs = !is(tunable("NHIP_BNB_L2_RUNS"), '0');
  p.general_all = is(tunable("NHIP_BNB_QUEUE"), '1');
  static_assert(NHIP_SHORT_SCAN_POINTS == 64 * OCL, "the header's promise is the by-rotation form's limit");
  p.short_scans = (search->flags & NHIP_SEARCH_SHORT_SCANS) != 0 && !p.general_all && (uint32_t)(L.S + 2 * L.pad) < ORG_LIMIT;
  p.instrumented = is(tunable("NHIP_BNB_INSTRUMENT"), '1');
  p.stats = p.instrumented && is(tunable("NHIP_BNB_STATS"), '1');
  p.timeline = p.instrumented && is(tunable("NHIP_BNB_TIMELINE"), '1');
  p.sized_split = n_pairs >= SPLIT_MIN_PAIRS || (n_pairs > 0 && (is(sp, '1') || sbat));
  if (workspace_bytes > 0 && n_pairs > 0 && !p.general_all && !is(sp, '0') && !is(force, '2') &&
      (n_pairs >= SPLIT_MIN_PAIRS || is(sp, '1'))) {
    p.batch = sbat && atoi(sbat) > 0 ? atoi(sbat) : SPLIT_PAIRS;
    if (p.batch > n_pairs) p.batch = n_pairs;
    for (;;) {
      p.slot_bytes = (split_state_bytes(p.batch, 1, search->n_theta) + 511) & ~(int64_t)511;
      p.slots = (workspace_bytes - BNB_WS_HEADER - 512) / p.slot_bytes;
      const int64_t rounds = (n_pairs + p.batch - 1) / p.batch;
      if (p.slots >= (rounds < 2 ? rounds : 2) || p.batch <= 512) break;
      p.batch = p.batch / 2 > 512 ? p.batch / 2 : 512;
    }
    if (p.slots > SPLIT_RING) p.slots = SPLIT_RING;
    if (p.slots < 1) p.batch = 0;
    if (!sbat && p.batch > 0 && n_pairs > p.batch && (p.slots < 2 || p.batch < SPLIT_PAIRS)) p.batch = 0;
  }
  p.rounds = p.batch > 0 ? (n_pairs + p.batch - 1) / p.batch : 1;
  if (p.batch > 0)
    p.form = !is(tunable("NHIP_BNB_SPLIT_OVERLAP"), '0') && p.slots >= 2 && n_pairs > p.batch
                 ? BNB_SPLIT_OVERLAP : (p.rounds > 1 ? BNB_SPLIT_ROUNDS : BNB_SPLIT_ONE);
  p.split_min = (uint32_t)std::max(num("NHIP_BNB_SPLIT_MIN", 300), 1);
  p.split_max = smax ? (uint32_t)std::max(atoi(smax), 1) : 0u;
  p.heavy_min = (uint32_t)num("NHIP_BNB_HEAVY_MIN", n_pairs <= 64 ? 1 : 384);
  p.keep_ranks = (uint32_t)num("NHIP_BNB_KEEP_RANKS", 8);
  const bool second = force ? force[0] == '2' : (n_pairs < 1024 && p.batch == 0 && (uint32_t)search->n_theta > p.keep_ranks);
  p.second = second && !p.general_all && workspace_bytes >= BNB_WS_HEADER + 8 * (int64_t)sizeof(RotEntry);
  if (p.second)
    p.rot_cap = (uint32_t)std::min<int64_t>((workspace_bytes - BNB_WS_HEADER) / (int64_t)sizeof(RotEntry) / 8, 0x0fffffff);
  p.pool_lds = bnb_lds_bytes(L, search, true) <= LDS_MAX;
  p.lds_first = (int64_t)bnb_lds_first(L, p.pool_lds);
  return p;
}

struct SplitSet {
  int device = -1;
  hipStream_t stream = nullptr;
  hipEvent_t ea[SPLIT_RING], eb[SPLIT_RING];
};
static std::mutex g_split_mu;
static std::vector<SplitSet *> g_split_free;

static int split_set_acquire(SplitSet **out) {
  int dev = -1;
  NHIP_TRY_HIP(hipGetDevice(&dev));
  {
    std::lock_guard<std::mutex> lock(g_split_mu);
    for (size_t i = 0; i < g_split_free.size(); i++)
      if (g_split_free[i]->device == dev) {
        *out = g_split_free[i];
        g_split_free.erase(g_split_free.begin() + (long)i);
        return NHIP_OK;
      }
  }
  SplitSet *n = new SplitSet();
  n->device = dev;
  hipError_t e = hipStreamCreateWithFlags(&n->stream, hipStreamNonBlocking);
  for (int i = 0; i < SPLIT_RING && e == hipSuccess; i++) {
    e = hipEventCreateWithFlags(&n->ea[i], hipEventDisableTiming);
    if (e == hipSuccess) e = hipEventCreateWithFlags(&n->eb[i], hipEventDisableTiming);
  }
  if (e != hipSuccess) {
    delete n;
    return hip_fail(e, "split form: helper stream / events", __FILE__, __LINE__);
  }
  *out = n;
  return NHIP_OK;
}
static void split_set_release(SplitSet *set) {
  if (!set) return;
  std::lock_guard<std::mutex> lock(g_split_mu);
  g_split_free.push_back(set);
}

static thread_local BnbPlan t_last_plan = {};
void bnb_last_launch(int32_t out[8]) {
  const BnbPlan &p = t_last_plan;
  const int32_t info[8] = {p.form, (int32_t)p.batch, (int32_t)p.slots, (int32_t)p.rounds, p.short_scans, p.second,
                           (int32_t)p.instrumented | ((int32_t)p.l2_runs << 1), p.n_pairs};
  memcpy(out, info, sizeof(info));
}

static void fill_bnb_params(BnbParams &P, const MatchJob &job, const BnbPlan &plan) {
  const GridLayout &L = *job.L;
  fill_job_params(P, job);
  P.pair_kbase = job.pair_kbase;
  P.keys = reinterpret_cast<unsigned long long *>(job.keys);
  P.gate = job_gate(job);
  P.nbx = (P.nx + BNB_B - 1) / BNB_B;
  P.nby = (P.ny + BNB_B - 1) / BNB_B;
  P.pool_pitch = L.pool_pitch;
  P.pool_rows = L.pool_rows;
  P.pairs_per_xcd = (plan.n_pairs + 7) / 8;
  P.skip_bytes = L.skip_bytes;
  P.pool_bytes = L.pool_bytes;
  P.pool4_bytes = L.pool4_bytes;
  P.pool4_pitch = L.pool4_pitch;
  P.hi_offset = L.hi_offset;
  P.hi_bytes = L.hi_bytes;
  P.hi_pitch = L.hi_pitch;
  P.hi_tpr = L.hi_tpr;
  P.hi_copy_bytes = L.hi_copy_bytes;
  P.t16_bytes = L.t16_bytes;
  P.t16_tpr = L.t16_tpr;
  P.inv_res_f = (float)P.inv_res;
  P.levels = plan.levels;
  P.l2_runs = plan.l2_runs;
  P.general_all = plan.general_all;
  P.short_scans = plan.short_scans;
  P.heavy_min = plan.heavy_min;
  P.keep_ranks = plan.keep_ranks;
  P.rot_cap = plan.rot_cap;
  P.lds_first = (int32_t)plan.lds_first;
}

static int instr_buffers(const BnbPlan &plan, BnbParams &P, hipStream_t s) {
  if (!plan.stats && !plan.timeline) return NHIP_OK;
  std::lock_guard<std::mutex> lock(g_instr_mu);
  if (plan.stats) {
    if (!g_bnb_stats) {
      NHIP_TRY_HIP(hipMalloc(reinterpret_cast<void **>(&g_bnb_stats), 8 * (BNB_STATS_HEAD + (size_t)BNB_STATS_PAIRS)));
      NHIP_TRY_HIP(hipMemset(g_bnb_stats, 0, 8 * (BNB_STATS_HEAD + (size_t)BNB_STATS_PAIRS)));
    }
    P.stats = g_bnb_stats;
  }
  if (plan.timeline) {
    if (!g_bnb_timeline) NHIP_TRY_HIP(hipMalloc(reinterpret_cast<void **>(&g_bnb_timeline), 48 * (size_t)BNB_STATS_PAIRS + 16));
    P.timeline = g_bnb_timeline;
    NHIP_TRY_HIP(hipMemsetAsync(g_bnb_timeline + 4 * (size_t)BNB_STATS_PAIRS + 2, 0xff, 8 * (size_t)BNB_STATS_PAIRS, s));
    NHIP_TRY_HIP(hipMemsetAsync(g_bnb_timeline + 5 * (size_t)BNB_STATS_PAIRS + 2, 0, 8 * (size_t)BNB_STATS_PAIRS, s));
    const unsigned long long init[2] = {~0ull, 0ull};
    NHIP_TRY_HIP(hipMemcpyAsync(g_bnb_timeline + 4 * (size_t)BNB_STATS_PAIRS, init, 16, hipMemcpyHostToDevice, s));
  }
  return NHIP_OK;
}

static int run_rounds(const BnbParams &P, const BnbPlan &plan, const BnbLaunchers &K, void *d_workspace,
                      int64_t workspace_bytes, hipStream_t s) {
  const bool overlap = plan.form == BNB_SPLIT_OVERLAP;
  SplitSet *set = nullptr;
  if (overlap) {
    const int rc = split_set_acquire(&set);
    if (rc) return rc;
  }
  std::unique_ptr<SplitSet, void (*)(SplitSet *)> set_guard(set, split_set_release);
  hipStream_t s2 = overlap ? set->stream : s;
  uint8_t *base = static_cast<uint8_t *>(d_workspace) + BNB_WS_HEADER;
  base += (512 - (reinterpret_cast<uintptr_t>(base) & 511)) & 511;
  int64_t round = 0;
  for (int64_t b0 = 0; b0 < plan.n_pairs; b0 += plan.batch, round++) {
    const int32_t nb = (int32_t)(plan.n_pairs - b0 < plan.batch ? plan.n_pairs - b0 : plan.batch);
    BnbParams Q = P;
    Q.pair_src += b0;
    Q.pair_slot += b0;
    Q.rot0_cs += 2 * b0;
    if (Q.pair_origin) Q.pair_origin += 2 * b0;
    Q.keys += b0;
    Q.pair_base = (int32_t)b0;
    Q.n_pairs = nb;
    Q.pairs_per_xcd = (nb + 7) / 8;
    Q.ps_work_stride = Q.pairs_per_xcd + (Q.pairs_per_xcd / 2 > 64 ? Q.pairs_per_xcd / 2 : 64);
    Q.split_min = plan.split_min;
    Q.split_max = plan.split_max ? plan.split_max : bnb_split_max(nb);
    Q.front_min = FRONT_MIN;
    uint8_t *w = base + (round % plan.slots) * plan.slot_bytes;
    Q.ps_count = reinterpret_cast<uint32_t *>(w);
    Q.ps_live = Q.ps_count + nb;
    Q.ps_next = Q.ps_live + nb;
    Q.ps_nw = Q.ps_next + nb;
    const bool spread = nb < SPREAD_BELOW_PAIRS;
    Q.ps_ticket = spread ? Q.ps_nw + nb : nullptr;
    Q.ps_work = reinterpret_cast<int32_t *>(Q.ps_nw + nb + 4);
    const uintptr_t rows = (reinterpret_cast<uintptr_t>(Q.ps_work + 8 * (size_t)Q.ps_work_stride) + 511) & ~(uintptr_t)511;
    Q.ps_rows = reinterpret_cast<uint32_t *>(rows);
    NHIP_REQUIRE((int64_t)(rows - reinterpret_cast<uintptr_t>(w)) + (int64_t)nb * P.n_theta * 512 <= plan.slot_bytes &&
                     w + plan.slot_bytes <= static_cast<uint8_t *>(d_workspace) + workspace_bytes,
                 "csm_bnb: workspace accounting");
    if (overlap && round >= plan.slots) NHIP_TRY_HIP(hipStreamWaitEvent(s, set->eb[(round - plan.slots) % SPLIT_RING], 0));
    NHIP_TRY_HIP(hipMemsetAsync(w, 0, 16 * (size_t)nb + 16, s));
    if (spread) NHIP_TRY_HIP(hipMemsetAsync(Q.ps_work, 0xff, 32 * (size_t)Q.ps_work_stride, s));
    {
      TimerScope t_a(NHIP_TIMER_CSM_BOUNDS, s);
      const int rc = K.split_a(Q, plan, s);
      if (rc) return rc;
    }
    if (overlap) {
      NHIP_TRY_HIP(hipEventRecord(set->ea[round % SPLIT_RING], s));
      NHIP_TRY_HIP(hipStreamWaitEvent(s2, set->ea[round % SPLIT_RING], 0));
    }
    {
      TimerScope t_b(NHIP_TIMER_CSM_CAND, s2);
      const int rc = K.split_b(Q, plan, s2);
      if (rc) return rc;
    }
    if (overlap) NHIP_TRY_HIP(hipEventRecord(set->eb[round % SPLIT_RING], s2));
  }
  if (overlap) NHIP_TRY_HIP(hipStreamWaitEvent(s, set->eb[(round - 1) % SPLIT_RING], 0));
  return NHIP_OK;
}

int launch_csm_bnb(const MatchJob &job) {
  const GridLayout &L = *job.L;
  const hipStream_t s = job.stream;
  NHIP_REQUIRE(bnb_fits(L, job.search), "csm_match: lattice %d x %d x %d beyond the branch-and-bound matcher's envelope",
               job.search->n_theta, job.search->nx, job.search->ny);
  if (job.n_pairs == 0) return NHIP_OK;
  const BnbPlan plan = bnb_plan(L, job.search, job.n_pairs, job.workspace ? job.workspace_bytes : 0);
  NHIP_REQUIRE(L.has_image || plan.short_scans, "csm_match: grids built with NHIP_GRID_NO_IMAGE serve lists whose scans all have at most %d "
               "points, and the caller must say so (NHIP_SEARCH_SHORT_SCANS; the handle API sets it itself)", NHIP_SHORT_SCAN_POINTS);
  BnbParams P;
  fill_bnb_params(P, job, plan);
  int rc = instr_buffers(plan, P, s);
  if (rc) return rc;
  if (plan.second) {
    P.rot_count = static_cast<uint32_t *>(job.workspace);
    P.rot_list = reinterpret_cast<RotEntry *>(static_cast<uint8_t *>(job.workspace) + BNB_WS_HEADER);
    NHIP_TRY_HIP(hipMemsetAsync(job.workspace, 0, BNB_WS_HEADER, s));
  }
  const BnbLaunchers K = plan.instrumented ? launchers_instr() : launchers_product();
  t_last_plan = plan;
  {
    TimerScope t_all(NHIP_TIMER_CSM, s);
    rc = plan.form == BNB_FUSED ? K.fused(P, plan, s) : run_rounds(P, plan, K, job.workspace, job.workspace_bytes, s);
  }
  if (rc) return rc;
  NHIP_TRY_HIP(hipGetLastError());
  launch_csm_finalize(job);
  NHIP_TRY_HIP(hipGetLastError());
  return NHIP_OK;
}

int bnb_stats_per_pair(unsigned long long *out, int32_t n) {
  if (!g_bnb_stats || n <= 0) return NHIP_OK;
  NHIP_TRY_HIP(hipMemcpy(out, g_bnb_stats + BNB_STATS_HEAD, 8 * (size_t)(n < BNB_STATS_PAIRS ? n : BNB_STATS_PAIRS), hipMemcpyDeviceToHost));
  return NHIP_OK;
}

int bnb_timeline_read(unsigned long long *out, int32_t n) {
  if (!g_bnb_timeline || n <= 0) return NHIP_OK;
  if (n > BNB_STATS_PAIRS) n = BNB_STATS_PAIRS;
  NHIP_TRY_HIP(hipMemcpy(out, g_bnb_timeline, 32 * (size_t)n, hipMemcpyDeviceToHost));
  NHIP_TRY_HIP(hipMemcpy(out + 4 * (size_t)n, g_bnb_timeline + 4 * (size_t)BNB_STATS_PAIRS, 16, hipMemcpyDeviceToHost));
  return NHIP_OK;
}

int bnb_timeline_cand_read(unsigned long long *out, int32_t n) {
  if (!g_bnb_timeline || n <= 0) return NHIP_OK;
  if (n > BNB_STATS_PAIRS) n = BNB_STATS_PAIRS;
  NHIP_TRY_HIP(hipMemcpy(out, g_bnb_timeline + 4 * (size_t)BNB_STATS_PAIRS + 2, 8 * (size_t)n, hipMemcpyDeviceToHost));
  NHIP_TRY_HIP(hipMemcpy(out + n, g_bnb_timeline + 5 * (size_t)BNB_STATS_PAIRS + 2, 8 * (size_t)n, hipMemcpyDeviceToHost));
  return NHIP_OK;
}

int bnb_stats_read(unsigned long long out[24]) {
  static_assert(BNB_STATS_HEAD == 24, "the head is what nhip_bnb_stats_levels hands out");
  for (int i = 0; i < BNB_STATS_HEAD; i++) out[i] = 0;
  if (!g_bnb_stats) return NHIP_OK;
  NHIP_TRY_HIP(hipMemcpy(out, g_bnb_stats, 8 * BNB_STATS_HEAD, hipMemcpyDeviceToHost));
  NHIP_TRY_HIP(hipMemset(g_bnb_stats, 0, 8 * BNB_STATS_HEAD));
  return NHIP_OK;
}


}
```

nautilus_amd/csrc/nhip_bnb_origin.h:

```cpp
#pragma once
#include "nhip_bnb_params.h"
#include "nhip_bnb_wave.h"

namespace nhip {
namespace {

using namespace bnb;

template <bool LEAN = false>
__device__ __forceinline__ void window_origin(float2 q, float cf, float sf, const BnbParams &P, int32_t cx, int32_t cy,
                                              int32_t *prow, int32_t *pcol) {
  const float xr = __fsub_rn(__fmul_rn(cf, q.x), __fmul_rn(sf, q.y));
  const float yr = __fadd_rn(__fmul_rn(sf, q.x), __fmul_rn(cf, q.y));
  const int32_t half = P.S / 2;
  const bool finite __attribute__((unused)) = (fabsf(xr) < 1e9f) && (fabsf(yr) < 1e9f);
  int32_t ix, iy;
  const float mx = __fmul_rn(xr, P.inv_res_f), my = __fmul_rn(yr, P.inv_res_f);
  const float fx = floorf(mx), fy = floorf(my);
  if (LEAN) {
    const float rx = __fsub_rn(mx, fx), ry = __fsub_rn(my, fy);
    const float dx = fminf(rx, __fsub_rn(1.0f, rx)), dy = fminf(ry, __fsub_rn(1.0f, ry));
    const float tx = __fmul_rn(fabsf(mx), 0x1p-22f), ty = __fmul_rn(fabsf(my), 0x1p-22f);
    const unsigned long long slow = __builtin_amdgcn_fcmpf(dx, tx, 13 ) | __builtin_amdgcn_fcmpf(dy, ty, 13 );
    ix = (int32_t)fx;
    iy = (int32_t)fy;
    const int32_t kx = half + cx - P.hx + P.pad, ky = half + cy - P.hy + P.pad;
    if (slow != 0ull) {
      const bool near_x = !(dx > tx), near_y = !(dy > ty);
      const bool big = (int)!(fabsf(mx) < 0x1p22f) | (int)!(fabsf(my) < 0x1p22f);
      const int32_t nx = (int32_t)rintf(mx), ny = (int32_t)rintf(my);
      const bool stay = (int)big | ((int)near_x & (int)(((nx + kx) & 7) == 0)) | ((int)near_y & (int)(((ny + ky) & 7) == 0));
      if (__builtin_amdgcn_ballot_w64(stay) != 0ull) {
        if (stay) {
          const double xd = (double)xr, yd = (double)yr;
          const bool fin = (fabs(xd) < 1e9) && (fabs(yd) < 1e9);
          ix = (int32_t)fmin(fmax(floor_quotient(xd, P.res, P.inv_res), -2147483000.0), 2147483000.0);
          iy = (int32_t)fmin(fmax(floor_quotient(yd, P.res, P.inv_res), -2147483000.0), 2147483000.0);
          if (!fin) ix = iy = -2147483000;
        }
      }
    }
    const int32_t lo_x = -P.hx - 1 - half - cx, lo_y = -P.hy - 1 - half - cy;
    ix = min(max(ix, lo_x), P.S + P.hx - half - cx);
    iy = min(max(iy, lo_y), P.S + P.hy - half - cy);
    *pcol = ix + kx;
    *prow = iy + ky;
    return;
  }
  const float rx = __fsub_rn(mx, fx), ry = __fsub_rn(my, fy);
  const bool near = fminf(rx, __fsub_rn(1.0f, rx)) <= __fmul_rn(fabsf(mx), 0x1p-22f) ||
                    fminf(ry, __fsub_rn(1.0f, ry)) <= __fmul_rn(fabsf(my), 0x1p-22f);
  ix = (int32_t)fx;
  iy = (int32_t)fy;
  if (__builtin_amdgcn_ballot_w64(near && finite) != 0ull) {
    if (near && finite) {
      ix = (int32_t)fmin(fmax(floor_quotient((double)xr, P.res, P.inv_res), -2147483000.0), 2147483000.0);
      iy = (int32_t)fmin(fmax(floor_quotient((double)yr, P.res, P.inv_res), -2147483000.0), 2147483000.0);
    }
  }
  ix = min(max(ix, -P.hx - 1 - half - cx), P.S + P.hx - half - cx);
  iy = min(max(iy, -P.hy - 1 - half - cy), P.S + P.hy - half - cy);
  const int32_t col = finite ? half + ix + cx : -P.hx - 1, row = finite ? half + iy + cy : -P.hy - 1;
  *pcol = col - P.hx + P.pad;
  *prow = row - P.hy + P.pad;
}

typedef uint32_t u32x2 __attribute__((ext_vector_type(2)));
typedef uint32_t u32x3 __attribute__((ext_vector_type(3)));
typedef uint32_t u32x4 __attribute__((ext_vector_type(4)));

__device__ __forceinline__ __amdgpu_buffer_rsrc_t uniform_rsrc(const void *base, int64_t bytes) {
  const uint64_t a = reinterpret_cast<uint64_t>(base);
  const uint32_t lo = (uint32_t)__builtin_amdgcn_readfirstlane((int)(uint32_t)a);
  const uint32_t hi = (uint32_t)__builtin_amdgcn_readfirstlane((int)(uint32_t)(a >> 32));
  const int n = __builtin_amdgcn_readfirstlane((int)(bytes < 0x7fffffffll ? bytes : 0x7fffffffll));
  return __builtin_amdgcn_make_buffer_rsrc(reinterpret_cast<void *>(((uint64_t)hi << 32) | lo), 0, n, 0x00020000);
}

__device__ __forceinline__ uint32_t idx_guard(bool live, uint32_t v) { return live ? v : 0u; }

__device__ __forceinline__ void rotation_k(const BnbParams &P, int32_t pair, int32_t k, float *cf, float *sf) {
  const double c0 = P.rot0_cs[2 * pair], s0 = P.rot0_cs[2 * pair + 1];
  const int32_t kd = k + (P.pair_kbase ? P.pair_kbase[pair] : 0);
  const double cd = P.delta_cs[2 * kd], sd = P.delta_cs[2 * kd + 1];
  *cf = __double2float_rn(__dsub_rn(__dmul_rn(c0, cd), __dmul_rn(s0, sd)));
  *sf = __double2float_rn(__dadd_rn(__dmul_rn(s0, cd), __dmul_rn(c0, sd)));
}

__device__ __forceinline__ void patch_origin(const BnbParams &P, bool live, float2 q, float cf, float sf, int32_t cx,
                                             int32_t cy, int32_t Y, int32_t X, uint32_t *g, uint32_t *sh) {
  *g = 0u;
  *sh = 0u;
  if (live) {
    int32_t prow, pcol;
    window_origin(q, cf, sf, P, cx, cy, &prow, &pcol);
    const int32_t col = pcol + BNB_B * X;
    *g = (uint32_t)((prow + BNB_B * Y) * P.pitch + (col & ~3));
    *sh = (uint32_t)(col & 3) * 8u;
  }
}


constexpr int ORG_COL_SHIFT = 6, ORG_ROW_SHIFT = 19;
__device__ __forceinline__ uint32_t org_row(uint32_t o) { return o >> ORG_ROW_SHIFT; }
__device__ __forceinline__ uint32_t org_col(uint32_t o) { return (o >> ORG_COL_SHIFT) & (ORG_LIMIT - 1u); }
__device__ __forceinline__ uint32_t org_cnt(uint32_t o) { return (o & 63u) + 1u; }

__device__ __forceinline__ uint32_t origin_of(const uint32_t *org, int c) { return c < OCL ? org[64 * c] : 0u; }

constexpr uint32_t RUN_KEY_MASK = (~0u << (ORG_ROW_SHIFT + 2)) | (((ORG_LIMIT >> 2) - 1u) << (ORG_COL_SHIFT + 2));
__device__ __forceinline__ uint32_t run_row2(uint32_t e) { return e >> (ORG_ROW_SHIFT + 2); }
__device__ __forceinline__ uint32_t run_col2(uint32_t e) { return (e >> (ORG_COL_SHIFT + 2)) & ((ORG_LIMIT >> 2) - 1u); }
__device__ __forceinline__ uint32_t run_cnt(uint32_t e) { return e & 127u; }
enum : int32_t { RUNS_NONE = 0, RUNS_FIELD = -1, RUNS_FULL = -2 };

template <bool RUNS = false, bool RING = RUNS>
__device__ __forceinline__ int32_t cache_origins(const BnbParams &P, const float2 *pts, int32_t n_pts, float cf, float sf,
                                                 int32_t cx, int32_t cy, int lane, uint32_t *org, bool merged,
                                                 uint32_t *runs = nullptr, bool want_runs = false,
                                                 int32_t *run_chunks = nullptr) {
  uint32_t *base = org - lane;
  const bool with_runs = RUNS && want_runs;
  if (RUNS) *run_chunks = RUNS_NONE;
  for (int merge = merged ? 1 : 0; merge >= 0; merge--) {
    constexpr int D = 3;
    uint32_t tail = 0u;
    uint32_t rtail = 0u;
    auto chunk = [&](float2 pt, int c) {
      const int32_t idx = 64 * c + lane;
      const bool live = idx < n_pts;
      uint32_t o = 0u;
      if (live) {
        int32_t prow, pcol;
        window_origin(pt, cf, sf, P, cx, cy, &prow, &pcol);
        o = ((uint32_t)prow << ORG_ROW_SHIFT) | ((uint32_t)pcol << ORG_COL_SHIFT);
      }
      const uint32_t prev = (uint32_t)__builtin_amdgcn_update_dpp((int)o, (int)o, 0x138 , 0xF, 0xF, false);
      const bool head = live && (lane == 0 || o != prev || merge == 0);
      const unsigned long long H = __ballot(head), L = __ballot(live);
      const unsigned long long rest = ((H | ~L) >> lane) >> 1;
      const uint32_t cnt = rest ? (uint32_t)__builtin_ctzll(rest) + 1u : (uint32_t)(64 - lane);
      if (head) {
        const uint32_t before = __builtin_amdgcn_mbcnt_hi((uint32_t)(H >> 32), __builtin_amdgcn_mbcnt_lo((uint32_t)H, 0u));
        base[tail + before] = o | (cnt - 1u);
      }
      tail += (uint32_t)__builtin_popcountll(H);
      if (RUNS && with_runs && merge) {
        const bool head2 = live && (lane == 0 || ((o ^ prev) & RUN_KEY_MASK) != 0u);
        const unsigned long long H2 = __ballot(head2);
        const unsigned long long rest2 = ((H2 | ~L) >> lane) >> 1;
        const uint32_t cnt2 = rest2 ? (uint32_t)__builtin_ctzll(rest2) + 1u : (uint32_t)(64 - lane);
        const uint32_t at = rtail + __builtin_amdgcn_mbcnt_hi((uint32_t)(H2 >> 32), __builtin_amdgcn_mbcnt_lo((uint32_t)H2, 0u));
        if (head2 && at < (uint32_t)RUN_WAVE) runs[at] = (o & RUN_KEY_MASK) | cnt2;
        rtail += (uint32_t)__builtin_popcountll(H2);
      }
    };
    const int32_t n_in = min(n_pts, 64 * OCL);
    if (RING) {
      constexpr int R = 6;
      float px[R], py[R];
#pragma unroll
      for (int d = 0; d < R; d++) {
        const float2 q = 64 * d + lane < n_pts ? pts[64 * d + lane] : make_float2(0.f, 0.f);
        px[d] = q.x;
        py[d] = q.y;
      }
#pragma unroll 1
      for (int c = 0; c < OCL; c++) {
        const int32_t idx = 64 * c + lane;
        if (64 * c >= n_pts) break;
        const float2 pt = make_float2(px[0], py[0]);
        const float2 qn = idx + 64 * R < n_pts ? pts[idx + 64 * R] : make_float2(0.f, 0.f);
#pragma unroll
        for (int d = 0; d < R - 1; d++) {
          px[d] = px[d + 1];
          py[d] = py[d + 1];
        }
        px[R - 1] = qn.x;
        py[R - 1] = qn.y;
        chunk(pt, c);
      }
    } else if (n_in > 0) {
      const uint32_t last = 8u * (uint32_t)(n_in - 1);
      auto point_at = [&](int32_t i) {
        return *reinterpret_cast<const float2 *>(reinterpret_cast<const char *>(pts) + min(8u * (uint32_t)i, last));
      };
      float2 q[D];
#pragma unroll
      for (int d = 0; d < D; d++) {
        int32_t i = 64 * d + lane;
        asm volatile("" : "+v"(i));
        q[d] = point_at(i);
        __builtin_amdgcn_sched_barrier(0);
      }
#pragma unroll 1
      for (int c = 0; 64 * c < n_in; c += D) {
#pragma unroll
        for (int d = 0; d < D; d++) {
          float2 pt = q[d];
          asm volatile("" : "+v"(pt.x), "+v"(pt.y));
          q[d] = point_at(64 * (c + d + D) + lane);
          if (d == 0 || 64 * (c + d) < n_in) chunk(pt, c + d);
        }
      }
    }
    const int32_t nch = (int32_t)((tail + 63u) >> 6);
    for (uint32_t e = tail + (uint32_t)lane; e < (uint32_t)ORG_WAVE; e += 64u) base[e] = 0u;
    if (RUNS && with_runs && merge)
      for (uint32_t e = rtail + (uint32_t)lane; e < (uint32_t)RUN_WAVE; e += 64u) runs[e] = 0u;
    __builtin_amdgcn_fence(__ATOMIC_RELEASE, "wavefront");
    __builtin_amdgcn_wave_barrier();
    if (merge == 0) {
      if (RUNS && with_runs) *run_chunks = RUNS_FIELD;
      return nch;
    }
    uint32_t w = 0u;
    for (int c = 0; c < nch; c++) {
      const uint32_t e = org[64 * c];
      w += 64u * (uint32_t)c + (uint32_t)lane < tail ? org_cnt(e) : 0u;
    }
    w = sum8(w);
    if (__ballot(w > 257u) == 0ull) {
      if (RUNS && with_runs) {
        const int32_t nrc = (int32_t)((rtail + 63u) >> 6);
        uint32_t w2 = 0u;
        if (rtail <= (uint32_t)RUN_WAVE)
          for (int c = 0; c < nrc; c++) w2 += run_cnt(runs[64 * c + lane]);
        w2 = sum8(w2);
        *run_chunks = rtail > (uint32_t)RUN_WAVE ? RUNS_FULL : (__ballot(w2 > 257u) != 0ull ? RUNS_FIELD : nrc);
      }
      return nch;
    }
    __builtin_amdgcn_wave_barrier();
  }
  return 0;
}

}
}
```

nautilus_amd/csrc/nhip_bnb_params.h:

```cpp
#pragma once
#include "nhip_common.h"
#include "nhip_csm_shared.h"

namespace nhip {
namespace bnb {

constexpr int BNB_WAVES = 8;
constexpr int NB = BNB_MAX_NB;
constexpr int MAX_ROT = 340;
constexpr int QCAP = 1024;
constexpr int SPLIT_WAVES = 8;
constexpr int LIST_ENTRIES = 128;
constexpr int RUN_SHIFT = 25;
constexpr int OC = 18;
constexpr int OCL = 17;
constexpr int ORG_WAVE = OCL * 64;
constexpr int ORG_LDS = BNB_WAVES * ORG_WAVE * 4;
constexpr uint32_t ORG_LIMIT = 1u << 13;
constexpr int RUN_CHUNKS = 8;
constexpr int RUN_WAVE = RUN_CHUNKS * 64;

constexpr int QSPACE_SPLIT = (SPLIT_WAVES * LIST_ENTRIES * 4 + MAX_ROT * 12 + 15) / 16 * 2;
constexpr int lds_qspace(bool split) { return split ? QSPACE_SPLIT : QCAP; }
static_assert(QSPACE_SPLIT <= QCAP, "the split form's LDS must not exceed the fused form's, which bnb_fits() checks");
struct LdsTail {
  unsigned long long best;
  uint32_t cnt[6];
  unsigned long long slow;
  uint32_t top;
};
constexpr int LDS_QN = 1, LDS_QHEAD = 2, LDS_TAIL_BYTES = 64;
static_assert(sizeof(LdsTail) <= LDS_TAIL_BYTES, "the tail fits its 64 bytes");
constexpr size_t lds_bytes(size_t first, int32_t n_theta, bool split) {
  return first + (size_t)n_theta * 128 * 4 + (size_t)lds_qspace(split) * 8 + LDS_TAIL_BYTES;
}

constexpr int BNB_STATS_PAIRS = 1 << 20;
constexpr int BNB_STATS_HEAD = 24;

struct RotEntry {
  unsigned long long w[4];
};

struct BnbParams {
  const float2 *xy;
  const int32_t *offsets;
  const uint8_t *grids;
  const int32_t *pair_src;
  const int32_t *pair_slot;
  IdBounds ids;
  const double *rot0_cs;
  const double *delta_cs;
  const int32_t *pair_origin;
  const int32_t *pair_kbase;
  unsigned long long *keys;
  unsigned long long *timeline;
  unsigned long long *stats;
  RotEntry *rot_list;
  uint32_t *rot_count;
  uint32_t rot_cap;
  uint32_t heavy_min;
  uint32_t keep_ranks;
  uint32_t *ps_rows;
  uint32_t *ps_count;
  uint32_t *ps_live;
  uint32_t *ps_next;
  uint32_t *ps_nw;
  int32_t *ps_work;
  uint32_t *ps_ticket;
  int32_t ps_work_stride;
  uint32_t split_min;
  uint32_t split_max;
  uint32_t front_min;
  int32_t pair_base;
  int32_t n_pairs, n_theta, nx, ny, hx, hy, nbx, nby;
  int32_t S, pad, pitch, rows, max_shift;
  int32_t pool_pitch, pool_rows, pairs_per_xcd;
  int32_t pool4_pitch;
  int32_t lds_first;
  int32_t general_all;
  int32_t short_scans;
  int32_t levels;
  int64_t grid_bytes, skip_bytes, slot_bytes, pool_bytes, pool4_bytes;
  int64_t hi_offset, hi_bytes;
  int32_t hi_pitch;
  int32_t hi_tpr;
  int64_t hi_copy_bytes;
  int64_t t16_bytes;
  int32_t t16_tpr;
  double res, inv_res;
  float inv_res_f;
  ScoreGate gate;
  int32_t l2_runs;
};

using BnbLaunch = int (*)(const BnbParams &P, const BnbPlan &plan, hipStream_t s);
struct BnbLaunchers { BnbLaunch fused, split_a, split_b; };
BnbLaunchers launchers_product();
BnbLaunchers launchers_instr();

}
}
```

nautilus_amd/csrc/nhip_common.h:

```cpp
#pragma once
#include <hip/hip_runtime.h>

#include <cmath>
#include <cstdint>
#include <cstdio>
#include <cstring>
#include <string>
#include <vector>

#include "../../include/nautilus_hip_debug.h"

namespace nhip {

void set_error(const char *fmt, ...);
int hip_fail(hipError_t e, const char *what, const char *file, int line);

#define NHIP_TRY_HIP(expr)                                            \
  do {                                                                \
    hipError_t _e = (expr);                                           \
    if (_e != hipSuccess) return ::nhip::hip_fail(_e, #expr, __FILE__, __LINE__); \
  } while (0)

#define NHIP_REQUIRE(cond, ...)          \
  do {                                   \
    if (!(cond)) {                       \
      ::nhip::set_error(__VA_ARGS__);    \
      return NHIP_ERR_ARG;               \
    }                                    \
  } while (0)

int require_device();

const char *tunable(const char *name);

struct IdBounds {
  int32_t n_scans;
  int32_t n_slots;
  uint32_t *status;
};
constexpr uint32_t BAD_TARGET_ID = 1u, BAD_PAIR_SRC = 2u, BAD_PAIR_SLOT = 4u, BAD_BLOCK_ID = 8u, BAD_POSE_ID = 16u,
                   BAD_SCAN_ID = 32u, BAD_FEATURE_IDX = 64u, BAD_FEATURE_COUNT = 128u, BAD_SCAN_OFFSETS = 256u,
                   BAD_MEMBER_ID = 512u, BAD_SUBMAP_CAPACITY = 1024u, BAD_CONTRIB_ID = 2048u, BAD_BLOCK_COLUMN = 4096u,
                   BAD_SYSTEM_ID = 8192u, BAD_MAP_SCAN_OFFSETS = 16384u, BAD_FREESPACE_PAIR = 32768u, BAD_PLACE_ID = 65536u;
constexpr int DEV_STATUS_WORDS = 4;
uint32_t *dev_status();
#ifdef __HIPCC__
__device__ __forceinline__ void flag_bad_id(uint32_t *status, uint32_t kind, int32_t value, int32_t index) {
  if (!status) return;
  if (atomicOr(status, kind) != 0u) return;
  status[1] = kind;
  status[2] = (uint32_t)value;
  status[3] = (uint32_t)index;
}
__device__ __forceinline__ bool id_in(int32_t id, int32_t n) { return (uint32_t)id < (uint32_t)n; }
__device__ __forceinline__ float float_norm_root(float d2) { return sqrtf(d2); }
__device__ __forceinline__ float float_norm(float dx, float dy) {
  return float_norm_root(__fadd_rn(__fmul_rn(dx, dx), __fmul_rn(dy, dy)));
}
__device__ __forceinline__ bool pair_ids_ok(const IdBounds &B, int32_t src, int32_t slot, int32_t pair, bool report) {
  const bool s_ok = id_in(src, B.n_scans), g_ok = id_in(slot, B.n_slots);
  if (s_ok && g_ok) return true;
  if (report) flag_bad_id(B.status, s_ok ? BAD_PAIR_SLOT : BAD_PAIR_SRC, s_ok ? slot : src, pair);
  return false;
}
#endif

constexpr int32_t GRID_MAX_SIDE = 16384;
struct GridLayout {
  int32_t S, pad, pitch, R;
  int32_t cb;
  int32_t levels;
  int64_t K;
  int64_t plain_bytes;
  bool has_image;
  int64_t grid_bytes;
  int64_t skip_bytes;
  int64_t pool_bytes;
  int64_t pool4_bytes;
  int64_t hi_bytes;
  int32_t hi_pitch;
  int32_t hi_tpr;
  int64_t hi_copy_bytes;
  int64_t t16_bytes;
  int32_t t16_tpr;
  int64_t hits_bytes;
  int32_t hits_pitch;
  int64_t slot_bytes;
  int64_t skip_offset;
  int64_t pool_offset;
  int64_t pool4_offset;
  int64_t hi_offset;
  int64_t t16_offset;
  int64_t hits_offset;
  int32_t pool_pitch, pool_rows;
  int32_t pool4_pitch, pool4_rows;
  double Lf, step;
};
constexpr uint32_t HI_TILE_BYTES = 128u;
__host__ __device__ __forceinline__ uint32_t hi_tiled(uint32_t row, uint32_t col, uint32_t cp, uint32_t tpr, uint32_t copy_bytes) {
  const uint32_t c = col + 8u * cp;
  return cp * copy_bytes + ((row >> 3) * tpr + (c >> 4)) * HI_TILE_BYTES + (row & 7u) * 16u + (c & 15u);
}

__host__ __device__ __forceinline__ uint32_t t16_tiled(uint32_t row, uint32_t col, uint32_t tpr) {
  return ((row >> 3) * tpr + (col >> 3)) * HI_TILE_BYTES + (row & 7u) * 16u + (col & 7u) * 2u;
}

constexpr int HIT_PAD = 32;

constexpr int BNB_B = 8;
constexpr int BNB_POOL = 2 * BNB_B - 1;
constexpr int BNB_MAX_NB = 11;
constexpr int BNB_B4 = 4;
constexpr int BNB_POOL4 = 2 * BNB_B4 - 1;
constexpr int CSM_WAVE_ROWS = 21;
constexpr int CSM_ROW_DW = 21;
#ifdef __HIPCC__
__device__ __forceinline__ double floor_quotient(double v, double res, double inv_res) {
  const double m = __dmul_rn(v, inv_res);
  double f = floor(m);
  const double frac = __dsub_rn(m, f);
  const double tol = __dmul_rn(fabs(m), 0x1p-50);
  if (frac <= tol || __dsub_rn(1.0, frac) <= tol) f = floor(__ddiv_rn(v, res));
  return f;
}
#endif

constexpr int64_t GRID_WS_HEADER = 256;
constexpr int64_t GRID_WS_THR16 = 65536 * 4;
constexpr int GRID_WS_MASK_WORDS = 5;
inline int64_t grid_ws_per_target(int32_t S) {
  const int64_t tiles = (S + 63) / 64;
  return (5 + 4 * GRID_WS_MASK_WORDS) * tiles * tiles;
}
__host__ __device__ constexpr int32_t skip_pitch(int32_t pitch) { return ((pitch / 4 + 63) / 64) * 8; }
int make_layout(const nhip_grid_spec_t *spec, GridLayout *L);

struct GridTables {
  int32_t taps[129];
  uint32_t thr[256];
  const uint32_t *thr16 = nullptr;
};
int make_tables(const nhip_grid_spec_t *spec, const GridLayout &L, GridTables *T);

void timer_begin(int id, hipStream_t s);
void timer_end(int id, hipStream_t s);

int launch_grid_build(const float *d_xy, const int32_t *d_offsets, int32_t n_scans, const int32_t *d_target_ids,
                      int32_t n_targets, const nhip_grid_spec_t *spec, const GridLayout &L,
                      uint8_t *d_grids, void *d_ws, int64_t ws_bytes, hipStream_t s, bool incremental = false);

enum MatchForm : int32_t {
  MATCH_BNB,
  MATCH_POSES,
  MATCH_STRIPS8,
  MATCH_STRIPS16,
};
struct MatchPlan {
  MatchForm form = MATCH_BNB;
  int32_t tile_rows = 0, n_tiles = 0;
  bool keys_zeroed = false, keys_undecoded = false;
};
MatchPlan csm_plan(const GridLayout &L, const nhip_search_t *search, int32_t n_pairs);

enum BnbForm : int32_t { BNB_FUSED, BNB_SPLIT_ONE, BNB_SPLIT_ROUNDS, BNB_SPLIT_OVERLAP };
struct BnbPlan {
  BnbForm form;
  int32_t n_pairs, cb, levels;
  bool second, general_all, short_scans, pool_lds, instrumented, stats, timeline;
  bool l2_runs;
  bool sized_split;
  uint32_t rot_cap, heavy_min, keep_ranks, split_min, split_max;
  int64_t batch, slots, slot_bytes, rounds;
  int64_t lds_first;
};
BnbPlan bnb_plan(const GridLayout &L, const nhip_search_t *search, int32_t n_pairs, int64_t workspace_bytes);

struct MatchJob {
  const float *xy = nullptr;
  const int32_t *offsets = nullptr;
  IdBounds ids = {0, 0, nullptr};
  const uint8_t *grids = nullptr;
  const nhip_grid_spec_t *spec = nullptr;
  const GridLayout *L = nullptr;
  const int32_t *pair_src = nullptr, *pair_slot = nullptr;
  const double *rot0_cs = nullptr;
  const double *delta_cs = nullptr;
  const int32_t *pair_origin = nullptr, *pair_kbase = nullptr;
  int32_t n_pairs = 0;
  const nhip_search_t *search = nullptr;
  double min_score = -INFINITY;
  uint64_t *keys = nullptr;
  nhip_match_t *out = nullptr;
  int32_t *sums = nullptr;
  hipStream_t stream = nullptr;
  void *workspace = nullptr;
  int64_t workspace_bytes = 0;
};

int launch_csm_match(const MatchJob &job, const MatchPlan &plan);

int launch_csm_bnb(const MatchJob &job);
int64_t bnb_workspace_bytes(int32_t n_pairs);
int64_t bnb_workspace_bytes_lists(int32_t n_pairs);
void bnb_last_launch(int32_t out[8]);
bool bnb_fits(const GridLayout &L, const nhip_search_t *search);
int bnb_stats_read(unsigned long long out[24]);
int bnb_timeline_read(unsigned long long *out, int32_t n);
int bnb_timeline_cand_read(unsigned long long *out, int32_t n);
int bnb_stats_per_pair(unsigned long long *out, int32_t n);
void launch_csm_finalize(const MatchJob &job);

int launch_csm_scores(const MatchJob &job, int32_t src, int32_t slot, int32_t origin_x, int32_t origin_y, int32_t *d_volume);

int launch_csm_exact_score(const MatchJob &job, const MatchPlan &plan);
bool csm_small_plane_fits(const nhip_search_t *search);
bool csm_small_tiled_fits(const nhip_search_t *search, int32_t n_pairs, int32_t *tile_rows, int32_t *n_tiles);
int launch_csm_small_match(const MatchJob &job, const MatchPlan &plan);
int launch_skipmap_build(uint8_t *d_grids, int32_t n_grids, const GridLayout &L, hipStream_t s);

int launch_resid_lidar(int kind, const float *d_corr, const int32_t *d_corr_block, int64_t n_corr,
                       const int32_t *d_block_src, const int32_t *d_block_tgt, int32_t n_blocks,
                       const double *d_poses, int32_t n_poses, double *d_block_consts,
                       double *d_res, double *d_jsrc, double *d_jtgt, hipStream_t s, double *d_jtgt_theta = nullptr,
                       int32_t block_base = 0, double *d_q = nullptr);

int launch_resid_normal_eq(int kind, const float *d_corr, const int32_t *d_block_offsets,
                           const int32_t *d_block_src, const int32_t *d_block_tgt, int32_t n_blocks,
                           const double *d_poses, int32_t n_poses, double *d_block_consts, double *d_out,
                           hipStream_t s);

int launch_corr_search(const float *d_xy, const float *d_normals, const int32_t *d_offsets, int32_t n_scans,
                       const int32_t *d_block_src, const int32_t *d_block_tgt, int32_t n_blocks,
                       const float *d_pose_aff, float thr, float min_cos, bool gate, const int64_t *d_cap_offsets,
                       float *d_corr_padded, int32_t *d_counts, hipStream_t s);

int launch_corr_compact(const float *d_corr_padded, const int64_t *d_cap_offsets,
                        const int32_t *d_counts, int32_t n_blocks, int32_t *d_block_offsets,
                        float *d_corr, int32_t *d_corr_block, hipStream_t s);

int launch_lc_scatter_scores(const float *d_xy, const int32_t *d_offsets, int32_t n_scans, double *d_scores, hipStream_t s);
int launch_lc_chi_square(const double *d_poses, int32_t n_poses, const int32_t *d_src, const int32_t *d_tgt, const float *d_cov,
                         int32_t n, double max_score, double *d_scores, uint8_t *d_flags, hipStream_t s);
int launch_lc_pair_gate(const double *d_poses, int32_t n_poses, const int32_t *d_cand, int32_t n, double max_range,
                        int32_t min_sep, uint8_t *d_flags, hipStream_t s);

int launch_round_norm(const float *d_dx, const float *d_dy, int64_t n, int32_t root_only, float *d_out, hipStream_t s);

int launch_feat_extract(const float *d_xy, const int32_t *d_offsets, int32_t n_scans, const nhip_feature_spec_t &spec,
                        int32_t *d_planar_idx, int32_t *d_planar_count, int32_t *d_edge_idx, int32_t *d_edge_count,
                        double *d_scores, hipStream_t s);
int launch_feat_pack(const float *d_xy, const float *d_normals, const int32_t *d_offsets, int32_t n_scans, const int32_t *d_idx,
                     const int32_t *d_count, int32_t cap, float *d_xy_out, float *d_normals_out, int32_t *d_offsets_out,
                     hipStream_t s);

int launch_submap_gather(const float *d_xy, const int32_t *d_offsets, int32_t n_scans, const int32_t *d_member_scan,
                         const float *d_member_affine, const int32_t *d_member_offsets, int32_t n_targets, float *d_out_xy,
                         int64_t out_capacity, int32_t *d_out_offsets, hipStream_t s);

int launch_normals_estimate(const float *d_xy, const int32_t *d_offsets, int32_t n_scans, const nhip_normals_spec_t &spec,
                            int32_t sample_limit, float *d_normals, int32_t *d_info, hipStream_t s);

struct VecState {
  int32_t stats[8];
  int32_t end;
  int32_t peak_t, peak_b, peak_votes;
  int32_t action;
  int32_t n_band;
};
enum { VEC_RETIRE = 1, VEC_COMMIT = 2 };
struct VecLayout {
  int64_t state, counts, cells, votes, live, row_off, tables, partial, bits, run_of_bin, run_lo, run_hi, run_slot, band_list, bytes;
  int32_t n_rho, n_along, bit_words, max_runs;
};
void vec_layout(const nhip_vectorize_spec_t &spec, int32_t max_cells, VecLayout *L);
struct VecParams {
  int32_t width, height, cell_x0, cell_y0, n_theta, n_rho, n_along, min_hits, min_votes, band_q, gap1, min_length, max_segments,
      max_cells, max_rounds, n_scans;
  double res, inv_res;
  VecState *st;
  int32_t *counts, *cells, *votes, *row_off, *run_of_bin, *run_lo, *run_hi, *run_slot, *band_list;
  const int32_t *C, *S;
  uint8_t *live;
  unsigned long long *partial;
  uint32_t *bits;
  long long *records;
  uint32_t *status;
};
int launch_vec_front(const VecParams &P, const float *d_xy, const int32_t *d_offsets, const float *d_affines, hipStream_t s);
int launch_vec_rounds(const VecParams &P, int32_t n, hipStream_t s);

struct OccParams {
  int32_t width, height, cell_x0, cell_y0, max_ray_cells, min_obs, occ_permille, free_permille, n_scans;
  double res, inv_res;
  int32_t *hits, *misses;
  int8_t *grid;
  long long *stats;
  uint32_t *status;
};
int launch_occupancy(const OccParams &P, bool clear, const float *d_xy, const int32_t *d_offsets, const float *d_affines,
                     hipStream_t s);

struct FsParams {
  const float2 *xy;
  const int32_t *offsets;
  const uint8_t *grids;
  uint8_t *free_planes;
  int32_t S, hits_pitch;
  int64_t slot_bytes, hits_offset, hits_bytes;
  double res, inv_res;
  IdBounds ids;
  const int32_t *target_ids;
  int32_t n_targets;
  const int32_t *pair_src, *pair_slot, *pair_origin;
  const double *rot0_cs, *delta_cs;
  const nhip_match_t *matches;
  int32_t *counts;
  int32_t n_pairs, pairs_per_xcd, n_theta, nx, ny, hx, hy, hit_radius, end_margin;
};
int launch_fs_trace(const FsParams &P, hipStream_t s);
int launch_fs_check(const FsParams &P, hipStream_t s);

constexpr int PLACE_MAX_RINGS = 32;
constexpr int PLACE_MATCH_MAX_RINGS = 15;
constexpr int PLACE_QT = 16;
struct PlaceTables {
  int32_t n_rings;
  float edge2[PLACE_MAX_RINGS + 1];
  float dir[64];
};
struct PlaceMatch {
  const unsigned long long *desc;
  const int32_t *bits;
  const int32_t *ids;
  uint16_t *keys;
  int32_t *records;
  long long *stats;
  uint32_t *status;
  int32_t n_scans, n_ids, pitch, n_rings, top_k, min_separation, max_permille, flags;
};
int launch_place_describe(const PlaceTables &T, const float *d_xy, const int32_t *d_offsets, int32_t n_scans, uint64_t *d_desc,
                          int32_t *d_bits, hipStream_t s);
int launch_place_match(const PlaceMatch &P, int32_t chunk_rows, hipStream_t s);

int launch_resid_point_to_line(const float *d_segments, const float *d_points,
                               const int32_t *d_point_block, int64_t n_points,
                               const int32_t *d_block_pose, const int32_t *d_block_line,
                               int32_t n_blocks, const double *d_poses, int32_t n_poses, const double *d_line_poses,
                               int32_t n_line_poses, double *d_res, double *d_jpose, double *d_jline, hipStream_t s);

int launch_resid_point_to_line_normal_eq(const float *d_segments, const float *d_points, const int32_t *d_block_offsets,
                                         const int32_t *d_block_pose, const int32_t *d_block_line, int32_t n_blocks,
                                         const double *d_poses, int32_t n_poses, const double *d_line_poses, int32_t n_line_poses,
                                         double *d_out, hipStream_t s);

int launch_hitl_select(const float *d_xy, const int32_t *d_offsets, int32_t n_scans, const float *d_pose_f32,
                       const nhip_hitl_spec_t &spec, uint8_t *d_class, int32_t *d_counts, int32_t *d_scan_block,
                       int32_t *d_scan_offset, int32_t *d_totals, hipStream_t s);
int launch_hitl_pack(const float *d_xy, const int32_t *d_offsets, int32_t n_scans, const uint8_t *d_class, const int32_t *d_counts,
                     const int32_t *d_scan_block, const int32_t *d_scan_offset, const int32_t *d_totals, int32_t n_blocks,
                     int32_t n_points, float *d_points, int32_t *d_block_offsets, int32_t *d_block_pose, hipStream_t s);

int launch_resid_odometry(const float *d_t_odom, const float *d_r_odom, const int32_t *d_pose_i,
                          const int32_t *d_pose_j, int32_t n_factors, double tw, double rw,
                          const double *d_poses, int32_t n_poses, double *d_res, double *d_ji, double *d_jj,
                          hipStream_t s);

int launch_resid_odometry_normal_eq(const float *d_t_odom, const float *d_r_odom, const int32_t *d_pose_i,
                                    const int32_t *d_pose_j, int32_t n_factors, double tw, double rw,
                                    const double *d_poses, int32_t n_poses, double *d_out, hipStream_t s);

struct PcgStats {
  int32_t done_a, done_b;
  int32_t iterations, flag;
  double relres, bb;
};
int launch_bsr_assemble(const double *d_rows, int32_t n_rows, const int32_t *d_row_ptr, const int32_t *d_col,
                        const int32_t *d_contrib_ptr, const int32_t *d_contrib, int32_t nb, int32_t nnzb, int32_t n_contrib,
                        double *d_values, double *d_grad, double *d_cost, hipStream_t s);
int64_t bsr_pcg_workspace_bytes(int32_t nb, int32_t nnzb);
int launch_bsr_pcg(const int32_t *d_row_ptr, const int32_t *d_col, const double *d_values, const double *d_grad,
                   const uint8_t *d_fixed, int32_t nb, int32_t nnzb, double lambda, double diag_floor, double tol,
                   int32_t first, int32_t last, bool final, double *d_x, void *d_ws, hipStream_t s);
int64_t bsr_pcg_columns_workspace_bytes(int32_t nb, int32_t nnzb, int32_t n_systems);
int launch_bsr_pcg_columns(const int32_t *d_row_ptr, const int32_t *d_col, const double *d_values, const uint8_t *d_fixed,
                           int32_t nb, int32_t nnzb, const int32_t *d_gauge, const int32_t *d_rhs_index, int32_t n_systems,
                           double ridge, double tol, int32_t first, int32_t last, bool final, double *d_x, void *d_ws,
                           hipStream_t s);
int bsr_pcg_columns_read(const void *d_ws, int32_t nb, int32_t n_systems, int32_t *n_active, int32_t *iters, int32_t *flag,
                         double *relres, hipStream_t s);

}
```

Before: 1.691 million.

## Add early-exit partial scoring for sub-block exact evaluation in branch-and-bound

Splits each scan's cached origin list at a cut chunk, pads both origins and runs so the first part is aligned, and records per-sub-block bounds for the remaining points during strip bounds. In exact sub-block scoring, it scores only the first part, adds the bound for the rest, and skips the sub-block if that cannot beat the current best. It also raises the default threshold for whole-block evaluation from 3 to 4 alive sub-blocks. The cost is extra padding, extra bound bookkeeping and reductions, a possible re-merge fallback, and more register pressure.

```diff
diff --git a/nautilus_amd/csm.py b/nautilus_amd/csm.py
--- a/nautilus_amd/csm.py
+++ b/nautilus_amd/csm.py
@@ -220,7 +220,8 @@
             "clk_slowest_wave": v[8], "clk_seeds": v[9], "clk_bounds": v[10], "clk_wave_phase3_100MHz": v[11],
             "pairs_handed_over": v[12], "clk_wave_second_kernel": v[13], "pose_evals16": v[14],
             "pairs_settled_by_gate": v[15], "passes_l2_runs": v[16], "passes_per_cell_field": v[17],
-            "passes_per_cell_capacity": v[18]}
+            "passes_per_cell_capacity": v[18], "early_exit_tested": v[19], "early_exit_stopped": v[20],
+            "passes_unsplit": v[21]}
 
 
 def score_volume(scans, grids, src, slot, theta0, search, origin=(0, 0)):
@@ -259,7 +260,7 @@
     form = {0: "fused", 1: "split, one round", 2: "split, rounds on one stream", 3: "split, rounds overlapped on the helper stream"}
     return {"form": form.get(out[0], "?"), "form_id": out[0], "pairs_per_round": out[1], "rounds_of_state": out[2],
             "rounds": out[3], "short_scans": bool(out[4]), "hand_over_kernel": bool(out[5]), "instrumented": bool(out[6] & 1),
-            "l2_runs": bool(out[6] & 2), "n_pairs": out[7]}
+            "l2_runs": bool(out[6] & 2), "early_exit": bool(out[6] & 4), "n_pairs": out[7]}
 
 
 def drop_in_cache_stats():
diff --git a/nautilus_amd/csrc/nhip_bnb.hip b/nautilus_amd/csrc/nhip_bnb.hip
--- a/nautilus_amd/csrc/nhip_bnb.hip
+++ b/nautilus_amd/csrc/nhip_bnb.hip
@@ -71,18 +71,19 @@
   n[0]++;
 }
 
-template <int CB, bool GLOBAL>
+template <int CB, bool GLOBAL, bool EE = false>
 __device__ __forceinline__ void process_candidate_c(const BnbParams &P, __amdgpu_buffer_rsrc_t rsrc, uint32_t pitch8,
                                                     __amdgpu_buffer_rsrc_t rsrc16, const uint32_t *org, int32_t nch,
                                                     int32_t n_pts, int32_t k, int32_t Y, int32_t X,
                                                     uint32_t sb0, uint32_t sb1, uint32_t sb2, uint32_t sb3, int lane,
-                                                    unsigned long long *best, uint32_t &bcopy, uint32_t (&n)[4]) {
+                                                    unsigned long long *best, uint32_t &bcopy, uint32_t (&n)[4],
+                                                    int32_t b_first = 0, uint32_t r0 = 0u, uint32_t r1 = 0u, uint32_t r2 = 0u,
+                                                    uint32_t r3 = 0u, uint32_t *ee = nullptr) {
   const uint32_t bsum = best_sum_cached<GLOBAL>(best, bcopy);
   const int alive = (sb0 != 0u && sb0 >= bsum) + (sb1 != 0u && sb1 >= bsum) + (sb2 != 0u && sb2 >= bsum) +
                     (sb3 != 0u && sb3 >= bsum);
   if (alive == 0) return;
-  constexpr int WHOLE_MIN = 3;
-  if (alive >= WHOLE_MIN) {
+  if (alive >= (EE ? P.whole_min : 3)) {
     int dy, dx;
     const uint32_t total = block_sums8(rsrc, pitch8, (uint32_t)P.hi_copy_bytes, org, nch, Y, X, lane, &dy, &dx);
     const int32_t ix = BNB_B * X + dx, iy = BNB_B * Y + dy;
@@ -99,9 +100,25 @@
 #pragma unroll 1
   for (int q = 0; q < 4; q++) {
     const uint32_t b = q == 0 ? sb0 : (q == 1 ? sb1 : (q == 2 ? sb2 : sb3));
-    if (b == 0u || b < best_sum_cached<GLOBAL>(best, bcopy)) continue;
+    const uint32_t bnow = best_sum_cached<GLOBAL>(best, bcopy);
+    if (b == 0u || b < bnow) continue;
     int dy, dx;
-    const uint32_t total = sub_sums8(rsrc, pitch8, (uint32_t)P.hi_copy_bytes, org, nch, Y, X, q >> 1, q & 1, lane, &dy, &dx);
+    uint32_t need = 0u;
+    bool stopped = false;
+    if (EE && b_first > 0) {
+      const uint32_t rest = q == 0 ? r0 : (q == 1 ? r1 : (q == 2 ? r2 : r3));
+      const uint32_t low = 255u * (uint32_t)n_pts;
+      const uint32_t lim = CB == 1 ? bnow : (bnow > low ? (bnow - low + 255u) >> 8 : 0u);
+      need = lim > rest ? lim - rest : 0u;
+    }
+    const int32_t b_test = EE && need != 0u ? b_first : 0;
+    const uint32_t total = sub_sums8<EE>(rsrc, pitch8, (uint32_t)P.hi_copy_bytes, org, nch, Y, X, q >> 1, q & 1, lane, &dy, &dx,
+                                         b_test, need, &stopped);
+    if (EE && BNB_STATS(P) && b_test > 0) {
+      ee[0]++;
+      ee[1] += stopped ? 1u : 0u;
+    }
+    if (EE && stopped) continue;
     const int32_t ix = BNB_B * X + BNB_B4 * (q & 1) + dx, iy = BNB_B * Y + BNB_B4 * (q >> 1) + dy;
     if (CB == 1) {
       const unsigned long long key = best_key(P, k, ix, iy, total, 8);
@@ -117,6 +134,7 @@
 struct PhaseClocks {
   long long org, strip, eval;
   uint32_t run_passes, cell_passes_field, cell_passes_full;
+  uint32_t ee[3];
 };
 
 __device__ __forceinline__ void flush_stats(unsigned long long *stats, const uint32_t *n, int32_t pair, const PhaseClocks *clk) {
@@ -134,6 +152,9 @@
     if (clk->run_passes) atomicAdd(&stats[16], (unsigned long long)clk->run_passes);
     if (clk->cell_passes_field) atomicAdd(&stats[17], (unsigned long long)clk->cell_passes_field);
     if (clk->cell_passes_full) atomicAdd(&stats[18], (unsigned long long)clk->cell_passes_full);
+#pragma unroll
+    for (int i = 0; i < 3; i++)
+      if (clk->ee[i]) atomicAdd(&stats[19 + i], (unsigned long long)clk->ee[i]);
   }
 }
 
@@ -147,12 +168,15 @@
   rotation_k(P, C.pair, k, &cf, &sf);
   if (BNB_STATS(P)) t_mark = clock64();
   int32_t nrc = RUNS_NONE;
-  const int32_t nch = cache_origins<RUNS>(P, C.pts, C.n_pts, cf, sf, C.cx, C.cy, lane, org, true, runs, RUNS && P.l2_runs != 0, &nrc);
+  int32_t split[2] = {0, 0};
+  const int32_t nch = cache_origins<RUNS>(P, C.pts, C.n_pts, cf, sf, C.cx, C.cy, lane, org, true, runs, RUNS && P.l2_runs != 0, &nrc,
+                                          RUNS ? min(P.ee_cut, EE_CUT_MAX) : 0, split);
   if (BNB_STATS(P)) clk.org += clock64() - t_mark;
   if (RUNS && BNB_STATS(P)) {
     clk.run_passes += nrc > 0 ? 1u : 0u;
     clk.cell_passes_field += nrc == RUNS_FIELD ? 1u : 0u;
     clk.cell_passes_full += nrc == RUNS_FULL ? 1u : 0u;
+    clk.ee[2] += P.ee_cut > 0 && split[0] == 0 ? 1u : 0u;
   }
   const __amdgpu_buffer_rsrc_t rsrc16 = CB == 1 ? uniform_rsrc(C.grid, P.grid_bytes + P.skip_bytes)
                                                 : uniform_rsrc(C.grid + P.hi_offset + 2 * P.hi_copy_bytes, P.t16_bytes);
@@ -169,10 +193,13 @@
       len++;
     }
     uint32_t sb[12];
+    uint32_t rest[12] = {0u, 0u, 0u, 0u, 0u, 0u, 0u, 0u, 0u, 0u, 0u, 0u};
     uint32_t bcopy = GLOBAL ? best_sum<true>(best) : 0u;
     if (P.levels >= 2) {
       if (BNB_STATS(P)) t_mark = clock64();
-      if (RUNS && nrc > 0) strip_bounds_c<RunList<RUN_CHUNKS>>(P, p4, runs + lane, nrc, Y, X0, len, CB == 1 ? 1u : 257u, sb);
+      if (RUNS && nrc > 0)
+        strip_bounds_c<RunList<RUN_CHUNKS>, RUNS>(P, p4, runs + lane, nrc, Y, X0, len, CB == 1 ? 1u : 257u, sb,
+                                                  split[0] > 0 ? split[1] : -1, rest);
       else strip_bounds_c<CellList>(P, p4, org, nch, Y, X0, len, CB == 1 ? 1u : 257u, sb);
       if (BNB_STATS(P)) clk.strip += clock64() - t_mark;
       n_work[1] += (uint32_t)len;
@@ -190,6 +217,12 @@
       const uint32_t s0 = t == 0 ? sb[0] : (t == 1 ? sb[4] : sb[8]), s1 = t == 0 ? sb[1] : (t == 1 ? sb[5] : sb[9]);
       const uint32_t s2 = t == 0 ? sb[2] : (t == 1 ? sb[6] : sb[10]), s3 = t == 0 ? sb[3] : (t == 1 ? sb[7] : sb[11]);
       if (BNB_STATS(P)) t_mark = clock64();
+      if (RUNS) {
+        const uint32_t r0 = t == 0 ? rest[0] : (t == 1 ? rest[4] : rest[8]), r1 = t == 0 ? rest[1] : (t == 1 ? rest[5] : rest[9]);
+        const uint32_t r2 = t == 0 ? rest[2] : (t == 1 ? rest[6] : rest[10]), r3 = t == 0 ? rest[3] : (t == 1 ? rest[7] : rest[11]);
+        process_candidate_c<CB, GLOBAL, true>(P, rsrc, pitch8, rsrc16, org, nch, C.n_pts, k, Y, X0 + t, s0, s1, s2, s3, lane, best,
+                                              bcopy, n_work, split[0], r0, r1, r2, r3, clk.ee);
+      } else
       process_candidate_c<CB, GLOBAL>(P, rsrc, pitch8, rsrc16, org, nch, C.n_pts, k, Y, X0 + t, s0, s1, s2, s3, lane, best,
                                       bcopy, n_work);
       if (BNB_STATS(P)) clk.eval += clock64() - t_mark;
@@ -337,7 +370,7 @@
   if (BY_ROT) {
     __syncthreads();
     uint32_t *org = s_org + wave * ORG_WAVE + lane;
-    PhaseClocks clk = {0, 0, 0, 0u, 0u, 0u};
+    PhaseClocks clk = {0, 0, 0, 0u, 0u, 0u, {0u, 0u, 0u}};
     long long t_busy = 0, t_wall = 0;
     const long long t_phase1 = BNB_STATS(P) ? clock64() : 0;
     if (BNB_TIMELINE(P) && threadIdx.x == 0 && pair < BNB_STATS_PAIRS) BNB_TIMELINE(P)[4 * pair + 1] = wall_clock64();
@@ -541,7 +574,7 @@
   __shared__ uint32_t s_run2[4 * RUN_WAVE];
   uint32_t *org = s_org2 + (threadIdx.x >> 6) * ORG_WAVE + lane;
   uint32_t *runs = s_run2 + (threadIdx.x >> 6) * RUN_WAVE;
-  PhaseClocks clk = {0, 0, 0, 0u, 0u, 0u};
+  PhaseClocks clk = {0, 0, 0, 0u, 0u, 0u, {0u, 0u, 0u}};
   const long long t0 = BNB_STATS(P) ? clock64() : 0;
   for (;;) {
     const uint32_t i = wave_fetch_add(P.rot_count + 8 * xcd + 1, 1u, lane);
@@ -680,7 +713,7 @@
   PairCtx C;
   pair_context(P, pair, &C);
   uint32_t n_work[4] = {0u, 0u, 0u, 0u};
-  PhaseClocks clk = {0, 0, 0, 0u, 0u, 0u};
+  PhaseClocks clk = {0, 0, 0, 0u, 0u, 0u, {0u, 0u, 0u}};
   const long long t0 = BNB_STATS(P) ? clock64() : 0;
   for (;;) {
     const uint32_t rank = wave_fetch_add(next, 1u, lane);
diff --git a/nautilus_amd/csrc/nhip_bnb_bounds.h b/nautilus_amd/csrc/nhip_bnb_bounds.h
--- a/nautilus_amd/csrc/nhip_bnb_bounds.h
+++ b/nautilus_amd/csrc/nhip_bnb_bounds.h
@@ -230,9 +230,10 @@
   static __device__ __forceinline__ uint32_t count(uint32_t e) { return run_cnt(e); }
 };
 
-template <class LIST>
+template <class LIST, bool REST = false>
 __device__ __forceinline__ void strip_sums(const BnbParams &P, __amdgpu_buffer_rsrc_t p4, const uint32_t *list, int32_t nch,
-                                           int32_t Y, int32_t X0, int len, uint32_t (&E)[3], uint32_t (&O)[3]) {
+                                           int32_t Y, int32_t X0, int len, uint32_t (&E)[3], uint32_t (&O)[3],
+                                           int32_t bstart, uint32_t (&EA)[3], uint32_t (&OA)[3]) {
   const uint32_t DP = (uint32_t)P.pool4_pitch;
   const uint32_t off = (uint32_t)(2 * Y) * DP + (uint32_t)(4 * X0);
   constexpr int ROUNDS = LIST::ROUNDS, H = LIST::H;
@@ -268,6 +269,13 @@
     }
 #pragma unroll
     for (int j = 0; j < H; j++) {
+      if (REST && H * h + j == bstart) {
+#pragma unroll
+        for (int t = 0; t < 3; t++) {
+          EA[t] = E[t];
+          OA[t] = O[t];
+        }
+      }
       const uint32_t n0 = __builtin_amdgcn_alignbit(w[j].y, w[j].x, sh[j]);
       const uint32_t n1 = __builtin_amdgcn_alignbit(w[j].z, w[j].y, sh[j]);
       const uint32_t n2 = __builtin_amdgcn_alignbit(w[j].w, w[j].z, sh[j]);
@@ -278,19 +286,33 @@
   }
 }
 
-template <class LIST>
+template <class LIST, bool REST = false>
 __device__ __forceinline__ void strip_bounds_c(const BnbParams &P, __amdgpu_buffer_rsrc_t p4, const uint32_t *list,
                                                int32_t nch, int32_t Y, int32_t X0, int len, uint32_t scale,
-                                               uint32_t (&out)[12]) {
+                                               uint32_t (&out)[12], int32_t bstart = -1, uint32_t *rest = nullptr) {
   uint32_t E[3] = {0u, 0u, 0u}, O[3] = {0u, 0u, 0u};
+  uint32_t EA[3] = {0u, 0u, 0u}, OA[3] = {0u, 0u, 0u};
   if (std::is_same<LIST, CellList>::value) {
-    strip_sums<CellList>(P, p4, list, nch, Y, X0, len, E, O);
+    strip_sums<CellList>(P, p4, list, nch, Y, X0, len, E, O, -1, EA, OA);
   } else {
     static_assert(RUN_CHUNKS == 8, "the rounds below cover the run list");
-    if (nch <= 4) strip_sums<RunList<4>>(P, p4, list, nch, Y, X0, len, E, O);
-    else if (nch == 5) strip_sums<RunList<5>>(P, p4, list, nch, Y, X0, len, E, O);
-    else if (nch == 6) strip_sums<RunList<6>>(P, p4, list, nch, Y, X0, len, E, O);
-    else strip_sums<RunList<8>>(P, p4, list, nch, Y, X0, len, E, O);
+    if (nch <= 4) strip_sums<RunList<4>, REST>(P, p4, list, nch, Y, X0, len, E, O, bstart, EA, OA);
+    else if (nch == 5) strip_sums<RunList<5>, REST>(P, p4, list, nch, Y, X0, len, E, O, bstart, EA, OA);
+    else if (nch == 6) strip_sums<RunList<6>, REST>(P, p4, list, nch, Y, X0, len, E, O, bstart, EA, OA);
+    else strip_sums<RunList<8>, REST>(P, p4, list, nch, Y, X0, len, E, O, bstart, EA, OA);
+  }
+  if (REST && bstart > 0) {
+    uint32_t r[12];
+#pragma unroll
+    for (int t = 0; t < 3; t++) {
+      const uint32_t e = sum8(E[t] - EA[t]), o = sum8(O[t] - OA[t]);
+      r[4 * t + 0] = e & 0xffffu;
+      r[4 * t + 1] = e >> 16;
+      r[4 * t + 2] = o & 0xffffu;
+      r[4 * t + 3] = o >> 16;
+    }
+#pragma unroll
+    for (int q = 0; q < 12; q++) rest[q] = wave_total_of8(r[q]);
   }
 #pragma unroll
   for (int t = 0; t < 3; t++) {
diff --git a/nautilus_amd/csrc/nhip_bnb_exact.h b/nautilus_amd/csrc/nhip_bnb_exact.h
--- a/nautilus_amd/csrc/nhip_bnb_exact.h
+++ b/nautilus_amd/csrc/nhip_bnb_exact.h
@@ -279,13 +279,64 @@
   return key;
 }
 
+template <bool EE = false>
 __device__ __forceinline__ uint32_t sub_sums8(__amdgpu_buffer_rsrc_t rsrc, uint32_t pitch, uint32_t copy_bytes, const uint32_t *org,
-                                              int32_t nch, int32_t Y, int32_t X, int32_t sy, int32_t sx, int lane, int *dy, int *dx) {
+                                              int32_t nch, int32_t Y, int32_t X, int32_t sy, int32_t sx, int lane, int *dy, int *dx,
+                                              int32_t b_first = 0, uint32_t need = 0u, bool *stopped = nullptr) {
   const uint32_t roff = (uint32_t)(BNB_B * Y + BNB_B4 * sy), coff = (uint32_t)(BNB_B * X + BNB_B4 * sx);
   const uint32_t wrap = pitch * HI_TILE_BYTES - HI_TILE_BYTES;
   constexpr int U = 2;
   static_assert(OC % U == 0, "whole rounds");
   uint32_t E[4] = {0u, 0u, 0u, 0u}, O[4] = {0u, 0u, 0u, 0u};
+  if (EE && b_first > 0) {
+    static_assert(EE_CUT_MAX % U == 0, "part A in whole rounds");
+#pragma unroll
+    for (int r = 0; r < EE_CUT_MAX / U; r++) {
+      if (U * r >= b_first) continue;
+      u32x2 w[U][4];
+      uint32_t sh[U], cn[U];
+#pragma unroll
+      for (int j = 0; j < U; j++) {
+        const uint32_t o = U * r + j < b_first ? org[64 * (U * r + j)] : 0u;
+        cn[j] = org_cnt(o);
+        const uint32_t row0 = org_row(o) + roff, col0 = org_col(o) + coff, col4 = col0 & ~3u;
+        const uint32_t cp = (col4 >> 3) & 1u, q = row0 & 7u;
+        const uint32_t v0 = hi_tiled(row0, col4, cp, pitch, copy_bytes);
+        sh[j] = (col0 & 3u) * 8u;
+#pragma unroll
+        for (int y = 0; y < 4; y++)
+          w[j][y] = __builtin_amdgcn_raw_buffer_load_b64(rsrc, (int)(v0 + (q + (uint32_t)y >= 8u ? wrap : 0u) + 16u * (uint32_t)y), 0, 0);
+      }
+#pragma unroll
+      for (int j = 0; j < U; j++)
+#pragma unroll
+        for (int y = 0; y < 4; y++) {
+          const uint32_t n = __builtin_amdgcn_alignbit(w[j][y].y, w[j][y].x, sh[j]);
+          E[y] += __umul24(n & M8, cn[j]);
+          O[y] += __umul24(n >> 8, cn[j]);
+        }
+    }
+    uint32_t R[8];
+#pragma unroll
+    for (int y = 0; y < 4; y++) {
+      R[2 * y] = E[y];
+      R[2 * y + 1] = O[y] - ((E[y] >> 16) << 8);
+    }
+    rs_step<8, 1>(R, lane & 1);
+    rs_step<4, 2>(R, lane & 2);
+    rs_step<2, 4>(R, lane & 4);
+    uint32_t V[2] = {R[0] & 0xffffu, R[0] >> 16};
+    rs_step<2, 8>(V, lane & 8);
+    V[0] = add_xor<16>(V[0]);
+    V[0] = add_xor<32>(V[0]);
+    const uint32_t m_a = (uint32_t)__builtin_amdgcn_readfirstlane((int)wave_max(V[0]));
+    if (m_a < need) {
+      *stopped = true;
+      return 0u;
+    }
+    org += 64 * b_first;
+    nch -= b_first;
+  }
 #pragma unroll
   for (int r = 0; r < OC / U; r++) {
     if (U * r >= nch) continue;
@@ -293,7 +344,7 @@
     uint32_t sh[U], cn[U];
 #pragma unroll
     for (int j = 0; j < U; j++) {
-      const uint32_t o = origin_of(org, U * r + j);
+      const uint32_t o = EE ? (U * r + j < nch ? org[64 * (U * r + j)] : 0u) : origin_of(org, U * r + j);
       cn[j] = org_cnt(o);
       const uint32_t row0 = org_row(o) + roff, col0 = org_col(o) + coff, col4 = col0 & ~3u;
       const uint32_t cp = (col4 >> 3) & 1u, q = row0 & 7u;
diff --git a/nautilus_amd/csrc/nhip_bnb_host.hip b/nautilus_amd/csrc/nhip_bnb_host.hip
--- a/nautilus_amd/csrc/nhip_bnb_host.hip
+++ b/nautilus_amd/csrc/nhip_bnb_host.hip
@@ -74,6 +74,9 @@
   p.cb = L.cb;
   p.levels = is(tunable("NHIP_BNB_LEVELS"), '1') ? 1 : 2;
   p.l2_runs = !is(tunable("NHIP_BNB_L2_RUNS"), '0');
+  p.early_exit = p.l2_runs && p.levels >= 2 && !is(tunable("NHIP_BNB_EARLY_EXIT"), '0');
+  p.ee_cut = std::min(std::max(num("NHIP_BNB_EE_CUT", EE_CUT), 1), EE_CUT_MAX);
+  p.whole_min = std::min(std::max(num("NHIP_BNB_WHOLE_MIN", 4), 1), 5);
   p.general_all = is(tunable("NHIP_BNB_QUEUE"), '1');
   static_assert(NHIP_SHORT_SCAN_POINTS == 64 * OCL, "the header's promise is the by-rotation form's limit");
   p.short_scans = (search->flags & NHIP_SEARCH_SHORT_SCANS) != 0 && !p.general_all && (uint32_t)(L.S + 2 * L.pad) < ORG_LIMIT;
@@ -157,7 +160,7 @@
 void bnb_last_launch(int32_t out[8]) {
   const BnbPlan &p = t_last_plan;
   const int32_t info[8] = {p.form, (int32_t)p.batch, (int32_t)p.slots, (int32_t)p.rounds, p.short_scans, p.second,
-                           (int32_t)p.instrumented | ((int32_t)p.l2_runs << 1), p.n_pairs};
+                           (int32_t)p.instrumented | ((int32_t)p.l2_runs << 1) | ((int32_t)p.early_exit << 2), p.n_pairs};
   memcpy(out, info, sizeof(info));
 }
 
@@ -186,6 +189,8 @@
   P.inv_res_f = (float)P.inv_res;
   P.levels = plan.levels;
   P.l2_runs = plan.l2_runs;
+  P.ee_cut = plan.early_exit ? plan.ee_cut : 0;
+  P.whole_min = plan.whole_min;
   P.general_all = plan.general_all;
   P.short_scans = plan.short_scans;
   P.heavy_min = plan.heavy_min;
diff --git a/nautilus_amd/csrc/nhip_bnb_origin.h b/nautilus_amd/csrc/nhip_bnb_origin.h
--- a/nautilus_amd/csrc/nhip_bnb_origin.h
+++ b/nautilus_amd/csrc/nhip_bnb_origin.h
@@ -118,11 +118,15 @@
 __device__ __forceinline__ int32_t cache_origins(const BnbParams &P, const float2 *pts, int32_t n_pts, float cf, float sf,
                                                  int32_t cx, int32_t cy, int lane, uint32_t *org, bool merged,
                                                  uint32_t *runs = nullptr, bool want_runs = false,
-                                                 int32_t *run_chunks = nullptr) {
+                                                 int32_t *run_chunks = nullptr, int32_t cut = 0, int32_t *split = nullptr) {
   uint32_t *base = org - lane;
   const bool with_runs = RUNS && want_runs;
   if (RUNS) *run_chunks = RUNS_NONE;
+  bool split_on = RUNS && RING && with_runs && cut > 0;
+  if (RUNS && RING && split) split[0] = split[1] = 0;
   for (int merge = merged ? 1 : 0; merge >= 0; merge--) {
+    uint32_t end_a = 0u, pad_a = 0u, rpad_a = 0u;
+    bool padded = false;
     constexpr int D = 3;
     uint32_t tail = 0u;
     uint32_t rtail = 0u;
@@ -178,6 +182,16 @@
         }
         px[R - 1] = qn.x;
         py[R - 1] = qn.y;
+        if (RUNS && split_on && merge && c == cut) {
+          end_a = tail;
+          pad_a = (tail + 63u) & ~63u;
+          if (tail + (uint32_t)lane < pad_a) base[tail + (uint32_t)lane] = 0u;
+          tail = pad_a;
+          rpad_a = (rtail + 63u) & ~63u;
+          if (rtail + (uint32_t)lane < rpad_a && rtail + (uint32_t)lane < (uint32_t)RUN_WAVE) runs[rtail + (uint32_t)lane] = 0u;
+          rtail = rpad_a;
+          padded = true;
+        }
         chunk(pt, c);
       }
     } else if (n_in > 0) {
@@ -217,7 +231,8 @@
     uint32_t w = 0u;
     for (int c = 0; c < nch; c++) {
       const uint32_t e = org[64 * c];
-      w += 64u * (uint32_t)c + (uint32_t)lane < tail ? org_cnt(e) : 0u;
+      const uint32_t i = 64u * (uint32_t)c + (uint32_t)lane;
+      w += i < tail && !(i >= end_a && i < pad_a) ? org_cnt(e) : 0u;
     }
     w = sum8(w);
     if (__ballot(w > 257u) == 0ull) {
@@ -229,9 +244,19 @@
         w2 = sum8(w2);
         *run_chunks = rtail > (uint32_t)RUN_WAVE ? RUNS_FULL : (__ballot(w2 > 257u) != 0ull ? RUNS_FIELD : nrc);
       }
-      return nch;
+      if (!(RUNS && RING && padded)) return nch;
+      if (*run_chunks > 0) {
+        split[0] = (int32_t)(pad_a >> 6);
+        split[1] = (int32_t)(rpad_a >> 6);
+        return nch;
+      }
     }
     __builtin_amdgcn_wave_barrier();
+    if (RUNS && RING && padded) {
+      split_on = false;
+      *run_chunks = RUNS_NONE;
+      merge = 2;
+    }
   }
   return 0;
 }
diff --git a/nautilus_amd/csrc/nhip_bnb_params.h b/nautilus_amd/csrc/nhip_bnb_params.h
--- a/nautilus_amd/csrc/nhip_bnb_params.h
+++ b/nautilus_amd/csrc/nhip_bnb_params.h
@@ -19,6 +19,7 @@
 constexpr uint32_t ORG_LIMIT = 1u << 13;
 constexpr int RUN_CHUNKS = 8;
 constexpr int RUN_WAVE = RUN_CHUNKS * 64;
+constexpr int EE_CUT = 7, EE_CUT_MAX = 10;
 
 constexpr int QSPACE_SPLIT = (SPLIT_WAVES * LIST_ENTRIES * 4 + MAX_ROT * 12 + 15) / 16 * 2;
 constexpr int lds_qspace(bool split) { return split ? QSPACE_SPLIT : QCAP; }
@@ -92,6 +93,8 @@
   float inv_res_f;
   ScoreGate gate;
   int32_t l2_runs;
+  int32_t whole_min;
+  int32_t ee_cut;
 };
 
 using BnbLaunch = int (*)(const BnbParams &P, const BnbPlan &plan, hipStream_t s);
diff --git a/nautilus_amd/csrc/nhip_common.h b/nautilus_amd/csrc/nhip_common.h
--- a/nautilus_amd/csrc/nhip_common.h
+++ b/nautilus_amd/csrc/nhip_common.h
@@ -169,6 +169,9 @@
   int32_t n_pairs, cb, levels;
   bool second, general_all, short_scans, pool_lds, instrumented, stats, timeline;
   bool l2_runs;
+  bool early_exit;
+  int32_t whole_min;
+  int32_t ee_cut;
   bool sized_split;
   uint32_t rot_cap, heavy_min, keep_ranks, split_min, split_max;
   int64_t batch, slots, slot_bytes, rounds;
```

Result: faster. 1.708 million, median of 6 (+1.0%).
